# hsinnan75/GSAlign

Hardware: AMD Instinct MI355X
Metric: aligned query Gbp/s (whole node) (higher is better)
Workload: dtype u8; 1 GPU; full-human-sized pair (BASELINE configs[4]): 24 contigs with GRCh38 chromosome lengths, 3.08 Gbp, repeat injection, vs 1; inflight_contexts_per_gpu=8, world_size=1, parallelism=one GPU

## Files before the change

### gsalign_amd/capi.py

```python
from __future__ import annotations

import ctypes as C
import os
import subprocess

import numpy as np

HERE = os.path.dirname(os.path.abspath(__file__))
LIB_PATH = os.path.join(HERE, "lib", "libgsa_hip.so")

EXPORTS = [
    "gsa_default_params", "gsa_create", "gsa_create_opts", "gsa_reserve_index", "gsa_release_reserved", "gsa_clone", "gsa_clone_to_device", "gsa_host_alloc", "gsa_host_free", "gsa_destroy", "gsa_set_params", "gsa_last_error", "gsa_align_contig", "gsa_align_many", "gsa_align_bundle",
    "gsa_align_contig_device", "gsa_set_query_device", "gsa_device_alloc", "gsa_device_free", "gsa_device_upload", "gsa_get_seed_stats", "gsa_hit_buffers", "gsa_seed_chunks", "gsa_hit_count", "gsa_export_hits", "gsa_import_hits", "gsa_finish_contig",
    "gsa_set_query", "gsa_rewind", "gsa_run_to", "gsa_seed_count", "gsa_get_seeds", "gsa_group_count", "gsa_get_groups", "gsa_get_blocks",
    "gsa_bwt_search_batch", "gsa_ksw2_batch", "gsa_gap_similarity_batch", "gsa_get_counters", "gsa_get_timings", "gsa_set_profiling", "gsa_bind_host_thread",
    "gsa_prefetch_contig", "gsa_prefetch_bundle", "gsa_cancel_prefetch", "gsa_get_wall_sums", "gsa_get_alloc_stats", "gsa_debug_buffers", "gsa_set_option", "gsa_host_register", "gsa_host_unregister",
    "gsa_call_variants", "gsa_align_many_variants", "gsa_get_variant_timing",
    "gsa_block_cigars", "gsa_get_cigar_timing", "gsa_align_many_ex",
    "gsa_block_cs", "gsa_get_cs_timing", "gsa_extras_cs",
    "gsa_lift_set", "gsa_lift", "gsa_get_lift_timing", "gsa_extras_lift",
    "gsa_track_set", "gsa_ref_track", "gsa_get_track_timing", "gsa_extras_track",
    "gsa_block_segs", "gsa_get_seg_timing", "gsa_extras_segs",
    "gsa_proj_open", "gsa_proj_close", "gsa_proj_clear", "gsa_project", "gsa_proj_fetch", "gsa_proj_merge", "gsa_get_proj_timing",
    "gsa_index_sizes", "gsa_build_index", "gsa_get_index_build_stats",
    "gsa_create_from_pac", "gsa_export_index_table",
]


class IndexView(C.Structure):
    _fields_ = [("primary", C.c_uint64), ("L2", C.c_uint64 * 5), ("bwt", C.POINTER(C.c_uint32)), ("bwt_words", C.c_uint64),
                ("sa", C.POINTER(C.c_uint64)), ("n_sa", C.c_uint64), ("ref", C.c_char_p), ("G", C.c_int64),
                ("chr_len", C.POINTER(C.c_int32)), ("n_chr", C.c_int32)]


class Params(C.Structure):
    _fields_ = [("min_seed_len", C.c_int32), ("max_indel", C.c_int32), ("min_block_score", C.c_int32), ("min_aln_len", C.c_int32),
                ("min_identity", C.c_int32), ("sensitive", C.c_int32), ("one_on_one", C.c_int32)]


class Seed(C.Structure):
    _fields_ = [("qpos", C.c_int32), ("len", C.c_int32), ("rpos", C.c_int64)]


class Frag(C.Structure):
    _fields_ = [("bseed", C.c_int32), ("qpos", C.c_int32), ("qlen", C.c_int32), ("rlen", C.c_int32), ("rpos", C.c_int64),
                ("aln_off", C.c_int64), ("aln_len", C.c_int32), ("_pad", C.c_int32)]


class Block(C.Structure):
    _fields_ = [("score", C.c_int32), ("aln_len", C.c_int32), ("bdup", C.c_int32), ("n_frag", C.c_int32), ("frag_off", C.c_int64),
                ("bdir", C.c_int32), ("gpos", C.c_int32), ("chr", C.c_int32), ("_pad", C.c_int32)]


class Rec(C.Structure):
    _fields_ = [("w0", C.c_int32), ("w1", C.c_int32), ("w2", C.c_int32), ("w3", C.c_uint32)]


class Result(C.Structure):
    _fields_ = [("n_blocks", C.c_int32), ("n_frags", C.c_int64), ("n_aln", C.c_int64), ("blocks", C.POINTER(Block)),
                ("recs", C.POINTER(Rec)), ("aln1", C.POINTER(C.c_char)), ("aln2", C.POINTER(C.c_char))]


class Variant(C.Structure):
    _fields_ = [("rpos", C.c_int64), ("qpos", C.c_int32), ("len", C.c_int32), ("chr", C.c_int32), ("pos", C.c_int32), ("kind", C.c_int32), ("block", C.c_int32)]


class Variants(C.Structure):
    _fields_ = [("n", C.c_int64), ("v", C.POINTER(Variant)), ("n_snv", C.c_int64), ("n_ins", C.c_int64), ("n_del", C.c_int64)]


VARIANT_DT = np.dtype([("rpos", "<i8"), ("qpos", "<i4"), ("len", "<i4"), ("chr", "<i4"), ("pos", "<i4"), ("kind", "<i4"), ("block", "<i4")])
VCF_TYPE = ("SUBSTITUTE", "INSERT", "DELETE", "INSERT", "DELETE")


def variants_array(var: "Variants"):
    n = int(var.n)
    V = np.ctypeslib.as_array(C.cast(var.v, C.POINTER(C.c_uint8)), shape=(n * VARIANT_DT.itemsize,)).view(VARIANT_DT).copy() if n else np.zeros(0, VARIANT_DT)
    return V, (int(var.n_snv), int(var.n_ins), int(var.n_del))


def variant_alleles(V: np.ndarray, ref, query) -> list:
    ref = ref.tobytes() if isinstance(ref, np.ndarray) else bytes(ref)
    query = query.tobytes() if isinstance(query, np.ndarray) else bytes(query)
    out = []
    for v in V:
        r, q, n, k = int(v["rpos"]), int(v["qpos"]), int(v["len"]) + 1, int(v["kind"])
        if k == 1:
            out.append((ref[r:r + 1], query[q:q + n]))
        elif k == 2:
            out.append((ref[r:r + n], query[q:q + 1]))
        elif k == 3:
            out.append((query[q:q + 1], query[q:q + n]))
        elif k == 4:
            out.append((ref[r:r + n], ref[r:r + 1]))
        else:
            out.append((ref[r:r + 1], query[q:q + 1]))
    return out


class BlockCigar(C.Structure):
    _fields_ = [("cig_off", C.c_int64), ("n_cig", C.c_int32), ("n_eq", C.c_int32), ("n_x", C.c_int32), ("n_ins", C.c_int32), ("n_del", C.c_int32), ("_pad", C.c_int32)]


class Cigars(C.Structure):
    _fields_ = [("n_blocks", C.c_int32), ("n_ops", C.c_int64), ("blk", C.POINTER(BlockCigar)), ("ops", C.POINTER(C.c_uint32))]


class Extras(C.Structure):
    _fields_ = [("var", C.POINTER(Variants)), ("cig", C.POINTER(Cigars))]


class CsBlock(C.Structure):
    _fields_ = [("cs_off", C.c_int64), ("n_cs", C.c_int32), ("_pad", C.c_int32)]


class Cs(C.Structure):
    _fields_ = [("n_blocks", C.c_int32), ("n_bytes", C.c_int64), ("blk", C.POINTER(CsBlock)), ("cs", C.POINTER(C.c_char))]


class LiftHit(C.Structure):
    _fields_ = [("idx", C.c_int32), ("qpos", C.c_int32), ("block", C.c_int32), ("cls", C.c_uint8), ("rev", C.c_uint8), ("n_cover", C.c_uint16)]


class Lifts(C.Structure):
    _fields_ = [("n_hits", C.c_int64), ("hits", C.POINTER(LiftHit))]


class TrackWin(C.Structure):
    _fields_ = [("chr", C.c_int32), ("start", C.c_int32), ("len", C.c_int32), ("n_cov", C.c_uint32), ("n_eq", C.c_uint32), ("n_x", C.c_uint32), ("n_del", C.c_uint32), ("n_ins", C.c_uint32)]


class Tracks(C.Structure):
    _fields_ = [("n_win", C.c_int64), ("win", C.POINTER(TrackWin))]


class Seg(C.Structure):
    _fields_ = [("size", C.c_int32), ("dt", C.c_int32), ("dq", C.c_int32)]


class SegBlock(C.Structure):
    _fields_ = [("seg_off", C.c_int64), ("n_seg", C.c_int32), ("_pad", C.c_int32)]


class Segs(C.Structure):
    _fields_ = [("n_blocks", C.c_int32), ("n_segs", C.c_int64), ("blk", C.POINTER(SegBlock)), ("seg", C.POINTER(Seg))]


SEG_DT = np.dtype([("size", "<i4"), ("dt", "<i4"), ("dq", "<i4")])
SEG_BLOCK_DT = np.dtype([("seg_off", "<i8"), ("n_seg", "<i4"), ("_pad", "<i4")])
TRACK_WIN_DT = np.dtype([("chr", "<i4"), ("start", "<i4"), ("len", "<i4"), ("n_cov", "<u4"), ("n_eq", "<u4"), ("n_x", "<u4"), ("n_del", "<u4"), ("n_ins", "<u4")])
LIFT_HIT_DT = np.dtype([("idx", "<i4"), ("qpos", "<i4"), ("block", "<i4"), ("cls", "u1"), ("rev", "u1"), ("n_cover", "<u2")])
BLOCK_CS_DT = np.dtype([("cs_off", "<i8"), ("n_cs", "<i4"), ("_pad", "<i4")])
BLOCK_CIGAR_DT = np.dtype([("cig_off", "<i8"), ("n_cig", "<i4"), ("n_eq", "<i4"), ("n_x", "<i4"), ("n_ins", "<i4"), ("n_del", "<i4"), ("_pad", "<i4")])
CIGAR_LETTERS = "MIDNSHP=X"
WANT_VARIANTS, WANT_CIGARS, WANT_CS, WANT_LIFT, WANT_TRACK, WANT_SEGS, WANT_PROJ = 1, 2, 4, 16, 32, 64, 128
PROJ_NO_DUP = 1
PROJ_LETTERS = "nACGTN-"


class ProjStat(C.Structure):
    _fields_ = [("n_blocks", C.c_int32), ("_pad", C.c_int32), ("n_cols", C.c_int64)]


def lifts_array(l: "Lifts"):
    n = int(l.n_hits)
    return np.ctypeslib.as_array(C.cast(l.hits, C.POINTER(C.c_uint8)), shape=(n * LIFT_HIT_DT.itemsize,)).view(LIFT_HIT_DT).copy() if n else np.zeros(0, LIFT_HIT_DT)
# ... 107 lines not shown
        if fn.argtypes is None:
            fn.argtypes = None
    return lib


def index_sizes(G: int):
    lib = load_library()
    lib.gsa_index_sizes.argtypes = [C.c_int64, C.POINTER(C.c_uint64), C.POINTER(C.c_uint64)]
    bw, ns = C.c_uint64(), C.c_uint64()
    rc = lib.gsa_index_sizes(int(G), C.byref(bw), C.byref(ns))
    if rc != 0:
        raise GsaError(f"gsa_index_sizes -> {rc}: {lib.gsa_last_error(None).decode()}")
    return int(bw.value), int(ns.value)


BUILD_INDEX_ARGTYPES = [C.c_int, C.c_void_p, C.c_int64, C.POINTER(C.c_uint64), C.POINTER(C.c_uint64), C.c_void_p, C.c_void_p]


def build_index_arrays(pac, G: int, device: int = 0):
    lib = load_library()
    lib.gsa_build_index.argtypes = BUILD_INDEX_ARGTYPES
    pac = np.ascontiguousarray(pac, dtype=np.uint8)
    if G <= 0 or pac.size < (G + 3) // 4:
        raise ValueError("pac holds fewer than G bases")
    bw, ns = index_sizes(G)
    bwt = np.zeros(bw, np.uint32); sa = np.zeros(ns, np.uint64)
    primary = C.c_uint64(); L2 = (C.c_uint64 * 5)()
    rc = lib.gsa_build_index(int(device), C.c_void_p(pac.ctypes.data), int(G), C.byref(primary), L2, C.c_void_p(bwt.ctypes.data), C.c_void_p(sa.ctypes.data))
    if rc != 0:
        e = GsaError(f"gsa_build_index -> {rc}: {lib.gsa_last_error(None).decode()}"); e.code = rc
        raise e
    return np.array([primary.value, L2[1], L2[2], L2[3], L2[4]], dtype=np.uint64), bwt, sa


def index_build_stats():
    lib = load_library()
    ms, rounds = C.c_double(), C.c_int32()
    lib.gsa_get_index_build_stats.argtypes = [C.POINTER(C.c_double), C.POINTER(C.c_int32)]
    lib.gsa_get_index_build_stats(C.byref(ms), C.byref(rounds))
    return float(ms.value), int(rounds.value)


def bind_host_thread(device: int = 0) -> None:
    lib = load_library()
    lib.gsa_bind_host_thread.argtypes = [C.c_int]
    lib.gsa_bind_host_thread(int(device))


RESULT_FN = C.CFUNCTYPE(C.c_int, C.c_void_p, C.c_int32, C.POINTER(Result))
RESULT_VAR_FN = C.CFUNCTYPE(C.c_int, C.c_void_p, C.c_int32, C.POINTER(Result), C.POINTER(Variants))
RESULT_EX_FN = C.CFUNCTYPE(C.c_int, C.c_void_p, C.c_int32, C.POINTER(Result), C.POINTER(Extras))


class DeviceContig:

    def __init__(self, lib, device: int, seq: np.ndarray):
        seq = np.ascontiguousarray(seq, dtype=np.uint8)
        self.lib, self.device, self.size = lib, int(device), int(seq.size)
        self.ptr = lib.gsa_device_alloc(self.device, self.size)
        if not self.ptr:
            raise GsaError("gsa_device_alloc failed")
        if lib.gsa_device_upload(self.device, C.c_void_p(self.ptr), C.c_void_p(seq.ctypes.data), self.size) != 0:
            raise GsaError("gsa_device_upload failed")

    def free(self):
        if self.ptr:
            self.lib.gsa_device_free(self.device, C.c_void_p(self.ptr)); self.ptr = None


def align_many(aligners, contigs, on_result=None, in_order: bool = False, bundle: bool = True, prefetch: bool = True, variants: bool = False, cigars: bool = False, cs: bool = False, lift: bool = False, track: bool = False, segs: bool = False, proj: bool = False) -> None:
    lib = aligners[0].lib
    n = len(contigs)
    ctxs = (C.c_void_p * len(aligners))(*[a.ctx for a in aligners])
    on_dev = n > 0 and isinstance(contigs[0], DeviceContig)
    qs = (C.c_char_p * n)(*[C.cast(c.ptr if on_dev else c.ctypes.data, C.c_char_p) for c in contigs])
    ql = (C.c_int32 * n)(*[int(c.size) for c in contigs])
    flags = (1 if in_order else 0) | (2 if on_dev else 0) | (0 if bundle else 8) | (0 if prefetch else 16)
    if cigars or cs or lift or track or segs or proj:
        lib.gsa_extras_cs.argtypes = [C.POINTER(Extras), C.POINTER(Cs)]
        lib.gsa_extras_lift.argtypes = [C.POINTER(Extras), C.POINTER(Lifts)]
        lib.gsa_extras_track.argtypes = [C.POINTER(Extras), C.POINTER(Tracks)]
        lib.gsa_extras_segs.argtypes = [C.POINTER(Extras), C.POINTER(Segs)]

        def ex_cb(user, ci, res, ex):
            e = ex.contents
            args = (ci, res.contents, e.var.contents if e.var else None, e.cig.contents if e.cig else None)
            if cs:
                s = Cs()
                rc_cs = lib.gsa_extras_cs(ex, C.byref(s))
                if rc_cs != 0:
                    return int(rc_cs)
                args += (s,)
            if lift:
                lf = Lifts()
                rc_l = lib.gsa_extras_lift(ex, C.byref(lf))
                if rc_l != 0:
                    return int(rc_l)
                args += (lf,)
            if track:
                tk = Tracks()
                rc_t = lib.gsa_extras_track(ex, C.byref(tk))
                if rc_t != 0:
                    return int(rc_t)
                args += (tk,)
            if segs:
                sg = Segs()
                rc_g = lib.gsa_extras_segs(ex, C.byref(sg))
                if rc_g != 0:
                    return int(rc_g)
                args += (sg,)
            return int((on_result(*args) if on_result else 0) or 0)
        cbx = RESULT_EX_FN(ex_cb)
        lib.gsa_align_many_ex.argtypes = [C.POINTER(C.c_void_p), C.c_int32, C.POINTER(C.c_char_p), C.POINTER(C.c_int32), C.c_int32, C.c_uint32, C.c_uint32, RESULT_EX_FN, C.c_void_p]
        rc = lib.gsa_align_many_ex(ctxs, len(aligners), qs, ql, n, flags, (WANT_CIGARS if cigars or cs else 0) | (WANT_CS if cs else 0) | (WANT_VARIANTS if variants else 0) | (WANT_LIFT if lift else 0) | (WANT_TRACK if track else 0) | (WANT_SEGS if segs else 0) | (WANT_PROJ if proj else 0), cbx, None)
    elif variants:
        cbv = RESULT_VAR_FN(lambda user, ci, res, var: int((on_result(ci, res.contents, var.contents) if on_result else 0) or 0))
        lib.gsa_align_many_variants.argtypes = [C.POINTER(C.c_void_p), C.c_int32, C.POINTER(C.c_char_p), C.POINTER(C.c_int32), C.c_int32, C.c_uint32, RESULT_VAR_FN, C.c_void_p]
        rc = lib.gsa_align_many_variants(ctxs, len(aligners), qs, ql, n, flags, cbv, None)
    else:
        cb = RESULT_FN((lambda user, ci, res: int(on_result(ci, res.contents) or 0)) if on_result else 0)
        lib.gsa_align_many.argtypes = [C.POINTER(C.c_void_p), C.c_int32, C.POINTER(C.c_char_p), C.POINTER(C.c_int32), C.c_int32, C.c_uint32, RESULT_FN, C.c_void_p]
        rc = lib.gsa_align_many(ctxs, len(aligners), qs, ql, n, flags, cb, None)
    if rc != 0:
        msgs = [lib.gsa_last_error(a.ctx).decode() for a in aligners]
        raise GsaError(f"gsa_align_many{'_ex' if cigars or cs or lift or track or segs or proj else '_variants' if variants else ''} -> {rc}: {'; '.join(m for m in msgs if m)}")


def _p(a, t):
    return a.ctypes.data_as(C.POINTER(t))


def result_as_dump(r: dict, with_aln: bool = False) -> dict:
    B, F = r["blocks"], r["frags"]
    idx = np.concatenate([np.arange(o, o + n) for o, n in zip(B["frag_off"], B["n_frag"])]) if B.size else np.zeros(0, np.int64)
    Fo = F[idx] if idx.size else np.zeros(0, FRAG_DT)
    out = {"b_score": B["score"].copy(), "b_aln_len": B["aln_len"].copy(), "b_bdup": B["bdup"].copy(), "b_nfrag": B["n_frag"].copy(),
           "b_bdir": B["bdir"].copy(), "b_gpos": B["gpos"].copy(), "b_chr": B["chr"].copy(),
           "f_bseed": Fo["bseed"].copy(), "f_qpos": Fo["qpos"].copy(), "f_qlen": Fo["qlen"].copy(), "f_rlen": Fo["rlen"].copy(),
           "f_alnlen": Fo["aln_len"].copy(), "f_rpos": Fo["rpos"].copy()}
    if with_aln:
        segs1 = [r["aln1"][o:o + n] for o, n in zip(Fo["aln_off"], Fo["aln_len"]) if n]
        segs2 = [r["aln2"][o:o + n] for o, n in zip(Fo["aln_off"], Fo["aln_len"]) if n]
        out["aln1"] = np.concatenate(segs1) if segs1 else np.zeros(0, np.uint8)
        out["aln2"] = np.concatenate(segs2) if segs2 else np.zeros(0, np.uint8)
    return out


class GsaError(RuntimeError):
    pass


class Aligner:

    ENV_OPTIONS = ("split_min", "bundle_contig", "bundle_cap", "seed_budget", "dp_lane", "seed_mode", "pd_bitmap", "walk_chain_min", "pd_two_level_min", "pres_from_kmer", "pd_bytes", "sweep_shape", "dp_side", "dp_safe", "dp_fake_timeout")

    def _options_from_env(self):
        for name in self.ENV_OPTIONS:
            v = os.environ.get("GSA_" + name.upper())
            if v is not None and v != "":
                self.set_option(name, {"sweep": 0, "spec": 1, "search": 2}.get(v, v) if name == "seed_mode" else v)
        if os.environ.get("GSA_NO_PDBITMAP"):
            self.set_option("pd_bitmap", 0)

    def set_option(self, name: str, value) -> None:
        self._ck(self.lib.gsa_set_option(self.ctx, name.encode(), C.c_int64(int(value))))

    def __init__(self, idx, device: int = 0, wide: bool = False, kmer_k: int = 0, pac=None, _clone_of=None, _copy_to=None, **params):
        self.lib = load_library()
        self.idx = idx
        self._pinned = []
        self._devbufs = []
        if _clone_of is not None and _copy_to is not None:
            self.ctx = C.c_void_p()
            rc = self.lib.gsa_clone_to_device(_clone_of.ctx, int(_copy_to), C.byref(self.ctx))
            if rc != 0:
                raise GsaError(f"gsa_clone_to_device -> {rc}: {self.lib.gsa_last_error(None).decode()}")
            self._options_from_env()
            return
        if _clone_of is not None:
            self.ctx = C.c_void_p()
            rc = self.lib.gsa_clone(_clone_of.ctx, C.byref(self.ctx))
            if rc != 0:
                raise GsaError(f"gsa_clone -> {rc}: {self.lib.gsa_last_error(None).decode()}")
            self._parent = _clone_of
            self._options_from_env()
            return
        self._ref = np.ascontiguousarray(idx.ref)
        v = IndexView()
        v.primary = int(idx.hdr[0])
        v.L2[0] = 0
        for i in range(1, 5):
            v.L2[i] = int(idx.hdr[i])
        v.bwt = _p(idx.bwt, C.c_uint32); v.bwt_words = idx.bwt.size
        v.sa = _p(idx.sa, C.c_uint64); v.n_sa = idx.sa.size
        v.ref = self._ref.ctypes.data_as(C.c_char_p); v.G = idx.G
        if pac is not None:
            self._pac = np.ascontiguousarray(pac, dtype=np.uint8)
            assert self._pac.size >= (idx.G + 3) // 4
            v.ref = self._pac.ctypes.data_as(C.c_char_p)
        v.chr_len = _p(idx.chr_len, C.c_int32); v.n_chr = len(idx.chr_len)
        self.ctx = C.c_void_p()
        p = self._params(**params)
        wide = wide or os.environ.get("GSA_FORCE_WIDE", "0") not in ("", "0")
        kmer_k = kmer_k or int(os.environ.get("GSA_KMER_K", "0") or 0)
        prio = int(os.environ.get("GSA_PRIO", "0") or 0)
        flags = (1 if wide else 0) | ((kmer_k & 15) << 8) | ((prio & 3) << 16) | (4 if pac is not None else 0)
        rc = self.lib.gsa_create_opts(device, C.byref(v), C.byref(p), flags, C.byref(self.ctx))
        if rc != 0:
            e = GsaError(f"gsa_create -> {rc}: {self.lib.gsa_last_error(None).decode()}"); e.code = rc
            raise e
        self._options_from_env()

    @classmethod
    def from_reference(cls, pac, G: int, chr_len, device: int = 0, wide: bool = False, kmer_k: int = 0, **params) -> "Aligner":
        self = cls.__new__(cls)
        self.lib = load_library()
        self.idx = None
        self._pinned = []
        self._devbufs = []
        self.lib.gsa_create_from_pac.argtypes = [C.c_int, C.c_void_p, C.c_int64, C.c_void_p, C.c_int32, C.POINTER(Params), C.c_uint32, C.POINTER(C.c_void_p)]
        pac = np.ascontiguousarray(pac, dtype=np.uint8); chr_len = np.ascontiguousarray(chr_len, dtype=np.int32)
        wide = wide or os.environ.get("GSA_FORCE_WIDE", "0") not in ("", "0")
        kmer_k = kmer_k or int(os.environ.get("GSA_KMER_K", "0") or 0)
        prio = int(os.environ.get("GSA_PRIO", "0") or 0)
        flags = (1 if wide else 0) | ((kmer_k & 15) << 8) | ((prio & 3) << 16)
        self.ctx = C.c_void_p()
        p = self._params(**params)
        rc = self.lib.gsa_create_from_pac(int(device), C.c_void_p(pac.ctypes.data), int(G), C.c_void_p(chr_len.ctypes.data), int(chr_len.size), C.byref(p), flags, C.byref(self.ctx))
        if rc != 0:
            e = GsaError(f"gsa_create_from_pac -> {rc}: {self.lib.gsa_last_error(None).decode()}"); e.code = rc
            raise e
        self._options_from_env()
        return self

    TABLES = {"header": 0, "occ": 1, "occ_base": 2, "sa_dense": 3, "sa": 4, "kmer": 5, "kmer_lo": 6, "pres": 7, "ref": 8, "ref2": 9}

    def index_table(self, which) -> np.ndarray:
        w = self.TABLES[which] if isinstance(which, str) else int(which)
        self.lib.gsa_export_index_table.argtypes = [C.c_void_p, C.c_int, C.c_void_p, C.c_uint64, C.POINTER(C.c_uint64)]
        n = C.c_uint64(0)
        self._ck(self.lib.gsa_export_index_table(self.ctx, w, None, 0, C.byref(n)))
        out = np.zeros(int(n.value), np.uint8)
        if out.size:
            self._ck(self.lib.gsa_export_index_table(self.ctx, w, C.c_void_p(out.ctypes.data), out.size, C.byref(n)))
        return out

    def clone(self) -> "Aligner":
        return Aligner(self.idx, _clone_of=self)

    def clone_to_device(self, device: int) -> "Aligner":
        return Aligner(self.idx, _clone_of=self, _copy_to=device)

    def pinned_copy(self, seq: np.ndarray) -> np.ndarray:
        seq = np.ascontiguousarray(seq, dtype=np.uint8)
        p = self.lib.gsa_host_alloc(seq.size + 64)
        if not p:
            raise GsaError("gsa_host_alloc failed")
        self._pinned.append(p)
        buf = np.ctypeslib.as_array(C.cast(p, C.POINTER(C.c_uint8)), shape=(seq.size,))
        buf[:] = seq
        return buf

    def device_copy(self, seq: np.ndarray, device: int = 0) -> DeviceContig:
        d = DeviceContig(self.lib, device, seq)
        self._devbufs.append(d)
        return d

    def prefetch_contig(self, seq: np.ndarray):
        self._ck(self.lib.gsa_prefetch_contig(self.ctx, seq.ctypes.data_as(C.c_char_p), C.c_int32(seq.size)))

    def cancel_prefetch(self):
        self._ck(self.lib.gsa_cancel_prefetch(self.ctx))

    def align_contig_device(self, d: DeviceContig) -> dict:
        res = Result()
        self._ck(self.lib.gsa_align_contig_device(self.ctx, C.c_void_p(d.ptr), C.c_int32(d.size), C.byref(res)))
        return self._result(res)

    def seed_stats(self) -> np.ndarray:
        st = np.zeros(8, np.uint64)
        self._ck(self.lib.gsa_get_seed_stats(self.ctx, _p(st, C.c_uint64)))
        return st

    def _params(self, slen=15, ind=25, clr=200, alen=200, idy=70, sen=0, one=0) -> Params:
        return Params(slen, ind, clr, alen, idy, sen, one)

    def _ck(self, rc):
        if rc != 0:
            raise GsaError(f"libgsa_hip error {rc}: {self.lib.gsa_last_error(self.ctx).decode()}")

    def set_params(self, **params):
        p = self._params(**params)
        self._ck(self.lib.gsa_set_params(self.ctx, C.byref(p)))

    def set_profiling(self, on: bool, count_blocks: bool = False, seed_only: bool = False, variants: bool = False):
        self._ck(self.lib.gsa_set_profiling(self.ctx, (1 if on else 0) | (2 if count_blocks else 0) | (4 if seed_only else 0) | (8 if variants else 0)))

    def set_query(self, seq: np.ndarray):
        seq = np.ascontiguousarray(seq, dtype=np.uint8)
        self._q = seq
        self._ck(self.lib.gsa_set_query(self.ctx, seq.ctypes.data_as(C.c_char_p), C.c_int32(seq.size)))

    def rewind(self):
        self._ck(self.lib.gsa_rewind(self.ctx))

    def run_to(self, stage: int):
        self._ck(self.lib.gsa_run_to(self.ctx, stage))

    def align_contig(self, seq: np.ndarray) -> dict:
        seq = np.ascontiguousarray(seq, dtype=np.uint8)
        self._q = seq
        res = Result()
        self._ck(self.lib.gsa_align_contig(self.ctx, seq.ctypes.data_as(C.c_char_p), C.c_int32(seq.size), C.byref(res)))
        return self._result(res)

    def seed_chunks(self, seq: np.ndarray, chunk_beg: int, chunk_end: int) -> int:
        seq = np.ascontiguousarray(seq, dtype=np.uint8)
        self._q = seq
        self._ck(self.lib.gsa_seed_chunks(self.ctx, seq.ctypes.data_as(C.c_char_p), C.c_int32(seq.size), C.c_int32(chunk_beg), C.c_int32(chunk_end)))
        return int(self.lib.gsa_hit_count(self.ctx))

    def hit_count(self) -> int:
        return int(self.lib.gsa_hit_count(self.ctx))

    def export_hits(self, keys_ptr=None, vals_ptr=None):
        n = int(self.lib.gsa_hit_count(self.ctx))
        if keys_ptr is not None:
            self._ck(self.lib.gsa_export_hits(self.ctx, C.c_void_p(keys_ptr), C.c_void_p(vals_ptr)))
            return n
        k = np.zeros(n, np.uint64); v = np.zeros(n, np.uint32)
        if n:
            self._ck(self.lib.gsa_export_hits(self.ctx, C.c_void_p(k.ctypes.data), C.c_void_p(v.ctypes.data)))
        return k, v

    def import_hits(self, keys, vals, n=None):
        if n is None:
            keys = np.ascontiguousarray(keys, np.uint64); vals = np.ascontiguousarray(vals, np.uint32)
            n = int(keys.size); kp, vp = keys.ctypes.data, vals.ctypes.data
        else:
            kp, vp = keys, vals
        self._ck(self.lib.gsa_import_hits(self.ctx, C.c_void_p(kp), C.c_void_p(vp), C.c_int64(n)))

    def finish_contig(self) -> dict:
        res = Result()
        self._ck(self.lib.gsa_finish_contig(self.ctx, C.byref(res)))
        return self._result(res)

    def seeds(self):
        n = self.lib.gsa_seed_count(self.ctx)
        out = np.zeros(n, dtype=SEED_DT)
        if n:
            self._ck(self.lib.gsa_get_seeds(self.ctx, out.ctypes.data_as(C.c_void_p)))
        return out["qpos"].copy(), out["len"].copy(), out["rpos"].copy()

    def groups(self):
        n = self.lib.gsa_group_count(self.ctx)
        b = np.zeros(n, np.int32); e = np.zeros(n, np.int32)
        if n:
            self._ck(self.lib.gsa_get_groups(self.ctx, _p(b, C.c_int32), _p(e, C.c_int32)))
        return b, e

    def _result(self, res: Result) -> dict:
        nb, nf, na = res.n_blocks, res.n_frags, res.n_aln
        blocks = np.ctypeslib.as_array(C.cast(res.blocks, C.POINTER(C.c_uint8)), shape=(nb * BLOCK_DT.itemsize,)).view(BLOCK_DT).copy() if nb else np.zeros(0, BLOCK_DT)
        recs = np.ctypeslib.as_array(C.cast(res.recs, C.POINTER(C.c_uint8)), shape=(nf * REC_DT.itemsize,)).view(REC_DT).copy() if nf else np.zeros(0, REC_DT)
        frags = expand_recs(recs)
        a1 = np.ctypeslib.as_array(C.cast(res.aln1, C.POINTER(C.c_uint8)), shape=(na,)).copy() if na else np.zeros(0, np.uint8)
        a2 = np.ctypeslib.as_array(C.cast(res.aln2, C.POINTER(C.c_uint8)), shape=(na,)).copy() if na else np.zeros(0, np.uint8)
        return dict(blocks=blocks, frags=frags, aln1=a1, aln2=a2)

    def call_variants(self, k: int = 0):
        var = Variants()
        self.lib.gsa_call_variants.argtypes = [C.c_void_p, C.c_int32, C.POINTER(Variants)]
        self._ck(self.lib.gsa_call_variants(self.ctx, C.c_int32(k), C.byref(var)))
        return variants_array(var)

    def block_cigars(self, k: int = 0):
        cig = Cigars()
        self.lib.gsa_block_cigars.argtypes = [C.c_void_p, C.c_int32, C.POINTER(Cigars)]
        self._ck(self.lib.gsa_block_cigars(self.ctx, C.c_int32(k), C.byref(cig)))
        return cigars_arrays(cig)

    def block_cs(self, k: int = 0):
        cs = Cs()
        self.lib.gsa_block_cs.argtypes = [C.c_void_p, C.c_int32, C.POINTER(Cs)]
        self._ck(self.lib.gsa_block_cs(self.ctx, C.c_int32(k), C.byref(cs)))
        return cs_arrays(cs)

    def lift_set(self, pos) -> None:
        pos = np.ascontiguousarray(pos, dtype=np.int64)
        self.lib.gsa_lift_set.argtypes = [C.c_void_p, C.c_void_p, C.c_int64]
        self._ck(self.lib.gsa_lift_set(self.ctx, C.c_void_p(pos.ctypes.data) if pos.size else None, C.c_int64(pos.size)))

    def lift(self, k: int = 0):
        l = Lifts()
        self.lib.gsa_lift.argtypes = [C.c_void_p, C.c_int32, C.POINTER(Lifts)]
        self._ck(self.lib.gsa_lift(self.ctx, C.c_int32(k), C.byref(l)))
        return lifts_array(l)

    def lift_timing(self):
        ms, n = C.c_double(0), C.c_int64(0)
        self.lib.gsa_get_lift_timing.argtypes = [C.c_void_p, C.POINTER(C.c_double), C.POINTER(C.c_int64)]
        self._ck(self.lib.gsa_get_lift_timing(self.ctx, C.byref(ms), C.byref(n)))
        return float(ms.value), int(n.value)

    def track_set(self, window: int) -> None:
        self.lib.gsa_track_set.argtypes = [C.c_void_p, C.c_int32]
        self._ck(self.lib.gsa_track_set(self.ctx, C.c_int32(int(window))))

    def track(self, k: int = 0):
        t = Tracks()
        self.lib.gsa_ref_track.argtypes = [C.c_void_p, C.c_int32, C.POINTER(Tracks)]
        self._ck(self.lib.gsa_ref_track(self.ctx, C.c_int32(k), C.byref(t)))
        return tracks_array(t)

    def track_timing(self):
        ms, n = C.c_double(0), C.c_int64(0)
        self.lib.gsa_get_track_timing.argtypes = [C.c_void_p, C.POINTER(C.c_double), C.POINTER(C.c_int64)]
        self._ck(self.lib.gsa_get_track_timing(self.ctx, C.byref(ms), C.byref(n)))
        return float(ms.value), int(n.value)

    def block_segs(self, k: int = 0):
        sg = Segs()
        self.lib.gsa_block_segs.argtypes = [C.c_void_p, C.c_int32, C.POINTER(Segs)]
        self._ck(self.lib.gsa_block_segs(self.ctx, C.c_int32(k), C.byref(sg)))
        return segs_arrays(sg)

    def seg_timing(self):
        ms, n = C.c_double(0), C.c_int64(0)
        self.lib.gsa_get_seg_timing.argtypes = [C.c_void_p, C.POINTER(C.c_double), C.POINTER(C.c_int64)]
        self._ck(self.lib.gsa_get_seg_timing(self.ctx, C.byref(ms), C.byref(n)))
        return float(ms.value), int(n.value)

    def proj_open(self, share: "Aligner" = None, no_dup: bool = False) -> None:
        self.lib.gsa_proj_open.argtypes = [C.c_void_p, C.c_void_p, C.c_uint32]
        self._ck(self.lib.gsa_proj_open(self.ctx, share.ctx if share is not None else None, C.c_uint32(PROJ_NO_DUP if no_dup else 0)))
# ... 160 lines not shown
```

### gsalign_amd/csrc/gsa_api.hip

```cpp
#include <cstring>
#include "gsa_ctx.h"

void collect_events(gsa_ctx *c)
{
	if (!c->profiling && !c->prof_seed) { c->ev_pending = 0; return; }
	float ms;
	if ((c->ev_pending & 1) && !c->profiling) {
		if (hipEventElapsedTime(&ms, c->ev[0], c->ev[1]) == hipSuccess) {
			c->kernel_ms[0] = ms;
			c->acc_seed_ms += ms;
		}
	} else {
		if (c->ev_pending & 1) {
			if (hipEventElapsedTime(&ms, c->ev[0], c->ev[1]) == hipSuccess) c->kernel_ms[0] = ms;
			if (hipEventElapsedTime(&ms, c->ev[1], c->ev[2]) == hipSuccess) c->kernel_ms[1] = ms;
			if (hipEventElapsedTime(&ms, c->ev[2], c->ev[3]) == hipSuccess) c->kernel_ms[2] = ms;
		}
		if (c->ev_pending & 2) { if (hipEventElapsedTime(&ms, c->ev[4], c->ev[5]) == hipSuccess) c->kernel_ms[3] = ms; }
	}
	c->ev_pending = 0;
	(void)hipGetLastError();
}

static int rewind_to_hits(gsa_ctx *c)
// ... 260 lines not shown
	if (n >= (1ll << 31) - 256) return gsa_fail(c, GSA_ERR_LIMIT, "gsa_lift_set: too many positions");
	for (int64_t i = 0; i < n; i++) if (pos[i] < 0 || pos[i] >= c->G)
		return gsa_fail(c, GSA_ERR_ARG, "gsa_lift_set: position " + std::to_string((long long)pos[i]) + " (entry " + std::to_string((long long)i) + ") lies outside the reference [0, " + std::to_string((long long)c->G) + ")");
	if (n == 0) { c->lift_n = 0; return GSA_OK; }
	GSA_CHECK(c, hipSetDevice(c->device));
	c->lift_n = 0;
	ENS(i64, d_lpos, (size_t)n);
	const hipError_t e = hipMemcpy(c->d_lpos.p, pos, (size_t)n * sizeof(i64), hipMemcpyHostToDevice);
	if (e != hipSuccess) { return gsa_fail(c, GSA_ERR_HIP, std::string("gsa_lift_set (hipMemcpy H2D): ") + hipGetErrorString(e)); }
	c->lift_n = n;
	return GSA_OK;
}
int gsa_lift(gsa_ctx *c, int32_t k, gsa_lifts *out) { return lift_call(c, k, out); }
int gsa_get_lift_timing(gsa_ctx *c, double *ms_sum, int64_t *n_calls) { return pass_timing(c, &gsa_ctx::lift_ms_sum, &gsa_ctx::lift_calls, ms_sum, n_calls); }

int gsa_track_set(gsa_ctx *c, int32_t window)
{
	if (!c) return GSA_ERR_ARG;
	if (window < 0) return gsa_fail(c, GSA_ERR_ARG, "gsa_track_set: the window is negative");
	i64 nwin = 0;
	if (window > 0) for (size_t i = 0; i < c->h_chr_len.size(); i++) nwin += ((i64)c->h_chr_len[i] + window - 1) / window;
	if (nwin >= (1ll << 31) - 256) return gsa_fail(c, GSA_ERR_LIMIT, "gsa_track_set: " + std::to_string((long long)nwin) + " windows (2^31 - 256 or more)");
	c->track_w = window; c->track_nwin = nwin;
	return GSA_OK;
}
int gsa_ref_track(gsa_ctx *c, int32_t k, gsa_tracks *out) { return track_call(c, k, out); }
int gsa_get_track_timing(gsa_ctx *c, double *ms_sum, int64_t *n_calls) { return pass_timing(c, &gsa_ctx::track_ms_sum, &gsa_ctx::track_calls, ms_sum, n_calls); }

int gsa_block_segs(gsa_ctx *c, int32_t k, gsa_segs *out) { return segs_call(c, k, out, nullptr, nullptr); }
int gsa_get_seg_timing(gsa_ctx *c, double *ms_sum, int64_t *n_calls) { return pass_timing(c, &gsa_ctx::seg_ms_sum, &gsa_ctx::seg_calls, ms_sum, n_calls); }

int gsa_proj_open(gsa_ctx *c, gsa_ctx *share, uint32_t flags) { return c ? proj_open(c, share, flags) : GSA_ERR_ARG; }
int gsa_proj_close(gsa_ctx *c)
{
	if (!c) return GSA_ERR_ARG;
	if (!c->proj) return gsa_fail(c, GSA_ERR_STATE, "gsa_proj_close: no accumulator (gsa_proj_open first)");
	return proj_release(c);
}
int gsa_proj_clear(gsa_ctx *c)
{
	if (!c) return GSA_ERR_ARG;
	if (!c->proj) return gsa_fail(c, GSA_ERR_STATE, "gsa_proj_clear: no accumulator (gsa_proj_open first)");
	return proj_clear(c);
}
int gsa_project(gsa_ctx *c, int32_t k, gsa_proj_stat *out) { return proj_call(c, k, out); }
static int proj_range_ready(gsa_ctx *c, int64_t p0, int64_t n, const char *who)
{
	if (!c) return GSA_ERR_ARG;
	if (!c->proj) return gsa_fail(c, GSA_ERR_STATE, std::string(who) + ": no accumulator (gsa_proj_open first)");
	if (n < 0 || p0 < 0 || p0 > c->proj->G || n > c->proj->G - p0) return gsa_fail(c, GSA_ERR_ARG, std::string(who) + ": the range lies outside the reference [0, " + std::to_string((long long)c->proj->G) + ")");
	return GSA_OK;
}
int gsa_proj_fetch(gsa_ctx *c, int64_t p0, int64_t n, char *text, uint32_t *words)
{
	if (const int rc = proj_range_ready(c, p0, n, "gsa_proj_fetch")) return rc;
	return (n == 0 || (!text && !words)) ? GSA_OK : proj_fetch(c, p0, n, text, words);
}
int gsa_proj_merge(gsa_ctx *c, int64_t p0, int64_t n, const uint32_t *words)
{
	if (const int rc = proj_range_ready(c, p0, n, "gsa_proj_merge")) return rc;
	if (n == 0) return GSA_OK;
	return words ? proj_merge(c, p0, n, words) : GSA_ERR_ARG;
}
int gsa_get_proj_timing(gsa_ctx *c, double *ms_sum, int64_t *n_calls) { return pass_timing(c, &gsa_ctx::proj_ms_sum, &gsa_ctx::proj_calls, ms_sum, n_calls); }

int gsa_get_wall_sums(gsa_ctx *c, double ms[10], int64_t *n)
{
	if (!c || !ms || !n) return GSA_ERR_ARG;
	memcpy(ms, c->wall_ms, sizeof(c->wall_ms)); *n = c->wall_n;
	if (c->up && c->own_up) { std::lock_guard<std::mutex> g(c->up->mu); ms[9] = c->up->jobs ? c->up->copy_ms / (double)c->up->jobs * (double)c->wall_n : 0.0; }
	return GSA_OK;
}
int gsa_get_alloc_stats(gsa_ctx *c, double *ms, int64_t *n, int64_t *bytes)
{
	if (!c) return GSA_ERR_ARG;
	if (ms) *ms = c->alloc_ms; if (n) *n = c->alloc_n; if (bytes) *bytes = c->alloc_bytes;
	return GSA_OK;
}

int gsa_set_profiling(gsa_ctx *c, int enable)
{
	if (!c) return GSA_ERR_ARG;
	c->acc_seed_ms = 0.0;
	memset(c->wall_ms, 0, sizeof(c->wall_ms));
	c->wall_n = 0;
	if (c->up && c->own_up) {
		std::lock_guard<std::mutex> g(c->up->mu);
		c->up->copy_ms = c->up->wait_ms = c->up->bytes = 0;
		c->up->jobs = 0;
	}
	c->var_ms_sum = 0;
	c->var_calls = 0;
	c->prof_var = (enable & 8) != 0;
	c->profiling = (enable & 1) != 0;
	c->count_blocks = (enable & 2) != 0;
	c->prof_seed = (enable & 4) != 0;
	return GSA_OK;
}

int64_t gsa_seed_count(gsa_ctx *c) { return c ? c->n_seeds : 0; }
int gsa_get_seeds(gsa_ctx *c, gsa_seed *out)
{
	if (!c || (!out && c->n_seeds)) return GSA_ERR_ARG;
	if (c->stage < 1) return gsa_fail(c, GSA_ERR_STATE, "run stage 1 first");
	const size_t n = (size_t)c->n_seeds; if (!n) return GSA_OK;
	{ int rc = seed_view_sort(c); if (rc) return rc; GSA_CHECK(c, hipStreamSynchronize(c->stream)); }
	std::vector<i32> q(n), l(n); std::vector<i64> r(n);
	GSA_CHECK(c, hipMemcpy(q.data(), c->s_q.p, n * 4, hipMemcpyDeviceToHost));
	GSA_CHECK(c, hipMemcpy(l.data(), c->s_len.p, n * 4, hipMemcpyDeviceToHost));
	GSA_CHECK(c, hipMemcpy(r.data(), c->s_r.p, n * 8, hipMemcpyDeviceToHost));
	for (size_t i = 0; i < n; i++) { out[i].qpos = q[i]; out[i].len = l[i]; out[i].rpos = r[i]; }
	return GSA_OK;
}
int gsa_group_count(gsa_ctx *c)
{
	if (!c) return 0;
	if (c->n_groups < 0) {
		if (seed_view_sort(c) != GSA_OK) return 0;
		hipStreamSynchronize(c->stream);
		i32 ng = 0;
		if (hipMemcpy(&ng, c->d_mail.as<i32>() + M_NG, 4, hipMemcpyDeviceToHost) != hipSuccess) return 0;
		c->n_groups = ng;
	}
	return c->n_groups;
}
int gsa_get_groups(gsa_ctx *c, int32_t *beg, int32_t *end)
{
	if (!c) return GSA_ERR_ARG;
	if (c->stage < 1) return gsa_fail(c, GSA_ERR_STATE, "run stage 1 first");
	const size_t ng = (size_t)gsa_group_count(c); if (!ng) return GSA_OK;
	std::vector<i32> gb(ng + 1);
	GSA_CHECK(c, hipMemcpy(gb.data(), c->g_beg.p, (ng + 1) * 4, hipMemcpyDeviceToHost));
	for (size_t i = 0; i < ng; i++) { beg[i] = gb[i]; end[i] = gb[i + 1]; }
	return GSA_OK;
}
int gsa_get_blocks(gsa_ctx *c, gsa_result *out)
{
	if (!c || !out) return GSA_ERR_ARG;
	if (c->stage < 2) return gsa_fail(c, GSA_ERR_STATE, "run stage 2 first");
	if (c->bnd.n && c->stage < 8) return gsa_fail(c, GSA_ERR_STATE, "gsa_get_blocks: the context holds a bundle -- only its finished result (gsa_align_bundle's out[]) is defined per contig");
	if (c->frags_stage != c->stage) { int rc = build_block_view(c); if (rc) return rc; }
	out->n_blocks = (int32_t)c->h_blocks.size(); out->blocks = c->h_blocks.data();
	if (c->result_pinned && c->stage == 8) {
		out->n_frags = c->n_frags; out->n_aln = c->n_aln;
		out->recs = c->p_frags.as<gsa_rec>(); out->aln1 = c->h_taln1; out->aln2 = c->h_taln2;
	} else {
		out->n_frags = (int64_t)c->h_frags.size(); out->n_aln = (int64_t)c->h_aln1.size();
		out->recs = c->h_frags.data(); out->aln1 = c->h_aln1.data(); out->aln2 = c->h_aln2.data();
	}
	return GSA_OK;
}
int gsa_get_counters(gsa_ctx *c, uint64_t counters[8]) { if (!c) return GSA_ERR_ARG; memcpy(counters, c->counters, sizeof(c->counters)); return GSA_OK; }
int gsa_get_timings(gsa_ctx *c, float ms[8]) { if (!c) return GSA_ERR_ARG; memcpy(ms, c->kernel_ms, sizeof(c->kernel_ms)); if (c->prof_seed && !c->profiling) ms[6] = (float)c->acc_seed_ms; return GSA_OK; }
int gsa_get_seed_stats(gsa_ctx *c, uint64_t st[8]) { if (!c) return GSA_ERR_ARG; memcpy(st, c->dbg, sizeof(c->dbg)); return GSA_OK; }
}
```

### gsalign_amd/csrc/gsa_create.hip

```cpp
#include <algorithm>
#include <cstring>
#include <pthread.h>
#include <sched.h>
#include "gsa_ctx.h"

static thread_local std::string g_create_error;
int gsa_fail(gsa_ctx *ctx, int code, const std::string &msg)
{
	if (ctx) ctx->err = msg; else g_create_error = msg;
	return code;
}

static int ctx_abandon(gsa_ctx *c, int rc, const std::string &msg = std::string())
{
	if (!msg.empty()) g_create_error = msg; else if (!c->err.empty()) g_create_error = c->err;
	gsa_destroy(c);
	return rc;
}

static int create_device_ok(const char *who, int device)
{
	int ndev = 0;
	if (hipGetDeviceCount(&ndev) != hipSuccess || ndev <= 0) { (void)hipGetLastError(); return gsa_fail(nullptr, GSA_ERR_HIP, "no HIP device available (libgsa_hip.so has no CPU path)"); }
	if (device < 0 || device >= ndev) return gsa_fail(nullptr, GSA_ERR_ARG, std::string(who) + ": bad device ordinal");
// ... 284 lines not shown
	(void)hipSetDeviceFlags(hipDeviceScheduleSpin); (void)hipGetLastError();
	gsa_ctx *c = new gsa_ctx();
	c->device = device; c->force_wide = parent->force_wide; c->prio_mode = parent->prio_mode; c->seed_budget = parent->seed_budget; c->opt = parent->opt;
	if (int rc = ctx_private_init(c)) return ctx_abandon(c, rc);
	struct Pair { const DevBuf *src; DevBuf *dst; };
	std::vector<Pair> tab = { { &own->d_bwt, &c->d_bwt }, { &own->d_occ_base, &c->d_occ_base }, { &own->d_sa, &c->d_sa }, { &own->d_ref, &c->d_ref }, { &own->d_chr_end, &c->d_chr_end },
		{ &own->d_chr_of_end, &c->d_chr_of_end }, { &own->d_sa_dense, &c->d_sa_dense }, { &own->d_kmer, &c->d_kmer }, { &own->d_ref2, &c->d_ref2 } };
	for (gsa_ctx *src = parent; src; src = src->lender) {
		if (!c->d_pres.cap && src->d_pres.p && (const void *)parent->di.pres == src->d_pres.p) { tab.push_back({ &src->d_pres, &c->d_pres }); c->d_pres.cap = 1; }
		if (!c->d_kmer_lo.cap && src->d_kmer_lo.p && (const void *)parent->di.kmer_lo == src->d_kmer_lo.p) { tab.push_back({ &src->d_kmer_lo, &c->d_kmer_lo }); c->d_kmer_lo.cap = 1; }
	}
	c->d_pres.cap = c->d_kmer_lo.cap = 0;
	for (const Pair &t : tab) {
		if (!t.src->p) continue;
		const size_t bytes = t.src->len ? t.src->len : t.src->cap;
		if (bytes == 0) return ctx_abandon(c, GSA_ERR_STATE, "gsa_clone_to_device: an index table of unknown size");
		if (hipMalloc(&t.dst->p, bytes + 256) != hipSuccess) { (void)hipGetLastError(); return ctx_abandon(c, GSA_ERR_NOMEM, "gsa_clone_to_device: hipMalloc of an index table"); }
		t.dst->cap = bytes + 256; t.dst->len = bytes;
		const hipError_t e = (device == own->device) ? hipMemcpyAsync(t.dst->p, t.src->p, bytes, hipMemcpyDeviceToDevice, c->stream)
		                                             : hipMemcpyPeerAsync(t.dst->p, device, t.src->p, own->device, bytes, c->stream);
		if (e != hipSuccess) return ctx_abandon(c, GSA_ERR_HIP, std::string("gsa_clone_to_device: device-to-device copy: ") + hipGetErrorString(e));
	}
	c->di = parent->di;
	auto move_ptr = [&](const void *p) -> const void * {
		if (!p) return nullptr;
		for (const Pair &t : tab) if (t.src->p && (const char *)p >= (const char *)t.src->p && (const char *)p < (const char *)t.src->p + (t.src->len ? t.src->len : t.src->cap)) return (const char *)t.dst->p + ((const char *)p - (const char *)t.src->p);
		return (const void *)~(uintptr_t)0;
	};
	bool lost = false;
#define MOVE(field, T) do { const void *q_ = move_ptr((const void *)c->di.field); if (q_ == (const void *)~(uintptr_t)0) lost = true; c->di.field = (T)q_; } while (0)
	MOVE(bwt, const uint4 *); MOVE(occ_base, const u64 *); MOVE(sa, const u64 *); MOVE(sa32, const u32 *); MOVE(sa64, const u64 *); MOVE(ref, const uint8_t *); MOVE(ref2, const u32 *);
	MOVE(chr_end, const i64 *); MOVE(chr_of_end, const i32 *); MOVE(kmer, const u64 *); MOVE(kmer_lo, const u64 *); MOVE(pres, const u32 *);
#undef MOVE
	if (lost) return ctx_abandon(c, GSA_ERR_STATE, "gsa_clone_to_device: an index pointer outside the tables of its owner");
	c->G = parent->G;
	c->h_chr_end = parent->h_chr_end; c->h_chr_fwd = parent->h_chr_fwd; c->h_chr_of_end = parent->h_chr_of_end; c->h_chr_len = parent->h_chr_len;
	c->prm = parent->prm;
	if (hipStreamSynchronize(c->stream) != hipSuccess) return ctx_abandon(c, GSA_ERR_HIP, "gsa_clone_to_device: waiting for the copies");
	*out = c;
	return GSA_OK;
}

int gsa_reserve_index(int device, uint64_t seq_len, uint32_t flags)
{
	int ndev = 0;
	if (hipGetDeviceCount(&ndev) != hipSuccess || device < 0 || device >= ndev || seq_len == 0) { (void)hipGetLastError(); return GSA_ERR_ARG; }
	if (hipSetDevice(device) != hipSuccess) return GSA_ERR_HIP;
	const bool wide = (flags & GSA_CREATE_WIDE) != 0 || seq_len >= 0xFFFFFFF0ull;
	size_t want[2];
	want[0] = ((size_t)seq_len + 1 + 32) * (wide ? 8 : 4) + 256;
	{
		int k = 0; while ((1ull << (2 * k)) < seq_len) k++;
		k += 2; if (k > 15) k = 15;
		size_t fr = 0, tot = 0; if (hipMemGetInfo(&fr, &tot) != hipSuccess) { (void)hipGetLastError(); fr = 8ull << 30; }
		const size_t esz = wide ? 32 : 16;
		while (k > 2 && ((size_t)esz << (2 * k)) > fr / 4) k--;
		const int kk = (int)((flags >> 8) & 15u); if (kk >= 2 && kk <= 15 && ((size_t)esz << (2 * kk)) <= fr / 2) k = kk;
		want[1] = k >= 2 ? ((size_t)esz << (2 * k)) : 0;
	}
	gsa_release_reserved(device);
	for (int k = 0; k < 2; k++) {
		if (!want[k]) continue;
		void *p = nullptr;
		if (hipMalloc(&p, want[k]) != hipSuccess) { (void)hipGetLastError(); continue; }
		std::lock_guard<std::mutex> g(g_res_mu);
		g_res[device & 63][k].p = p; g_res[device & 63][k].bytes = want[k];
	}
	return GSA_OK;
}
void gsa_release_reserved(int device)
{
	void *f[2] = { nullptr, nullptr };
	{ std::lock_guard<std::mutex> g(g_res_mu); for (int k = 0; k < 2; k++) { f[k] = g_res[device & 63][k].p; g_res[device & 63][k].p = nullptr; g_res[device & 63][k].bytes = 0; } }
	if (f[0] || f[1]) { (void)hipSetDevice(device); for (int k = 0; k < 2; k++) if (f[k]) hipFree(f[k]); }
}

static bool device_local_cpus(int device, cpu_set_t *set)
{
	char bus[64] = { 0 };
	if (hipDeviceGetPCIBusId(bus, (int)sizeof(bus) - 1, device) != hipSuccess) { (void)hipGetLastError(); return false; }
	for (char *p = bus; *p; p++) if (*p >= 'A' && *p <= 'Z') *p = (char)(*p - 'A' + 'a');
	char path[160]; snprintf(path, sizeof(path), "/sys/bus/pci/devices/%s/local_cpulist", bus);
	FILE *f = fopen(path, "r"); if (!f) return false;
	char line[4096]; const bool got = fgets(line, sizeof(line), f) != nullptr; fclose(f);
	if (!got) return false;
	CPU_ZERO(set); int n = 0;
	for (char *p = line; *p;) {
		while (*p == ',' || *p == ' ' || *p == '\n') p++;
		if (!*p) break;
		char *e; long a = strtol(p, &e, 10), b = a; if (e == p) break;
		if (*e == '-') { p = e + 1; b = strtol(p, &e, 10); if (e == p) break; }
		for (long k = a; k <= b && k < CPU_SETSIZE; k++) { CPU_SET((int)k, set); n++; }
		p = e;
	}
	return n > 0;
}
int gsa_bind_host_thread(int device)
{
	cpu_set_t set;
	if (!device_local_cpus(device, &set)) return GSA_OK;
	(void)pthread_setaffinity_np(pthread_self(), sizeof(set), &set);
	return GSA_OK;
}

void *gsa_host_alloc(size_t bytes)
{
	void *p = nullptr;
	if (hipHostMalloc(&p, bytes ? bytes : 1) != hipSuccess) { (void)hipGetLastError(); return nullptr; }
	return p;
}
void gsa_host_free(void *p) { if (p) (void)hipHostFree(p); }
int gsa_host_register(void *p, size_t bytes)
{
	if (!p || !bytes) return GSA_ERR_ARG;
	if (hipHostRegister(p, bytes, hipHostRegisterDefault) != hipSuccess) { (void)hipGetLastError(); return GSA_ERR_HIP; }
	return GSA_OK;
}
int gsa_host_unregister(void *p)
{
	if (!p) return GSA_ERR_ARG;
	if (hipHostUnregister(p) != hipSuccess) { (void)hipGetLastError(); return GSA_ERR_HIP; }
	return GSA_OK;
}

void *gsa_device_alloc(int device, size_t bytes)
{
	void *p = nullptr;
	if (hipSetDevice(device) != hipSuccess || hipMalloc(&p, (bytes ? bytes : 1) + 64) != hipSuccess) { (void)hipGetLastError(); return nullptr; }
	return p;
}
void gsa_device_free(int device, void *p) { if (p && hipSetDevice(device) == hipSuccess) (void)hipFree(p); }
int gsa_device_upload(int device, void *dst, const void *src, size_t bytes)
{
	if (!dst || (!src && bytes)) return GSA_ERR_ARG;
	if (hipSetDevice(device) != hipSuccess || hipMemcpy(dst, src, bytes, hipMemcpyHostToDevice) != hipSuccess) { (void)hipGetLastError(); return GSA_ERR_HIP; }
	return GSA_OK;
}

int gsa_set_option(gsa_ctx *c, const char *name, int64_t value)
{
	if (!c || !name) return GSA_ERR_ARG;
	const std::string k(name);
	auto in = [&](int64_t lo, int64_t hi) { return value >= lo && value <= hi; };
	const int64_t BIG = (int64_t)1 << 40;
	if (k == "split_min") { if (!in(0, BIG)) return gsa_fail(c, GSA_ERR_ARG, "split_min: 0 .. 2^40 bases"); c->opt.split_min = value; }
	else if (k == "bundle_contig") { if (!in(0, BIG)) return gsa_fail(c, GSA_ERR_ARG, "bundle_contig: 0 (no bundles) .. 2^40 bases"); c->opt.bundle_contig = value; }
	else if (k == "bundle_cap") { if (!in(1, BIG)) return gsa_fail(c, GSA_ERR_ARG, "bundle_cap: 1 .. 2^40 bases"); c->opt.bundle_cap = value; }
	else if (k == "seed_budget") { if (!in(1, 0xffffffffll)) return gsa_fail(c, GSA_ERR_ARG, "seed_budget: 1 .. 2^32 - 1 wave-iterations"); c->seed_budget = (u32)value; }
	else if (k == "dp_lane") { if (!in(0, 1 << 20)) return gsa_fail(c, GSA_ERR_ARG, "dp_lane: 0 (no lane class: one per wavefront) .. 2^20 cells"); c->opt.dp_lane = (int)value; }
	else if (k == "seed_mode") { if (value < 0 || value > 2) return gsa_fail(c, GSA_ERR_ARG, "seed_mode: 0 sweep, 1 speculative, 2 search"); c->opt.seed_mode = (int)value; }
	else if (k == "seed_lhop") { if (value != 0 && (!in(16, 1 << 16) || (value & (value - 1)))) return gsa_fail(c, GSA_ERR_ARG, "seed_lhop: 0 or a power of two >= 16"); c->opt.seed_lhop = (int)value; }
	else if (k == "pd_bitmap") c->opt.pd_bitmap = value != 0;
	else if (k == "dp_side") c->opt.dp_side = value != 0;
	else if (k == "pd_two_level_min") { if (!in(0, BIG)) return gsa_fail(c, GSA_ERR_ARG, "pd_two_level_min: >= 0 blocks"); c->opt.pd_two_level_min = value; }
	else if (k == "pd_bytes") { if (!in(0, 2)) return gsa_fail(c, GSA_ERR_ARG, "pd_bytes: 0 never, 1 by the hit count, 2 always"); c->opt.pd_bytes = (int)value; }
	else if (k == "pres_from_kmer") c->opt.pres_from_kmer = value != 0;
	else if (k == "walk_chain_min") { if (!in(0, BIG)) return gsa_fail(c, GSA_ERR_ARG, "walk_chain_min: >= 0 seeds"); c->opt.walk_chain_min = value; }
	else if (k == "sweep_shape") { if (value < -1 || value > 1) return gsa_fail(c, GSA_ERR_ARG, "sweep_shape: -1, 0 or 1"); c->opt.sweep_shape = (int)value; }
	else if (k == "dp_safe") c->dp_safe = value != 0;
	else if (k == "dp_fake_timeout") { if (!in(0, 1 << 20)) return gsa_fail(c, GSA_ERR_ARG, "dp_fake_timeout: >= 0"); c->dp_fake_timeout = (int)value; }
	else return gsa_fail(c, GSA_ERR_ARG, "gsa_set_option: unknown option " + k);
	return GSA_OK;
}

int gsa_debug_buffers(gsa_ctx *c, int top)
{
	if (!c) return GSA_ERR_ARG;
	struct E { const char *name; size_t cap, len; };
	std::vector<E> v;
#define X(n) if (c->n.p) v.push_back({ #n, c->n.cap, c->n.len });
	GSA_DEVBUFS(X)
#undef X
	std::sort(v.begin(), v.end(), [](const E &a, const E &b) { return a.cap > b.cap; });
	size_t tot = 0; for (const E &e : v) tot += e.cap;
	fprintf(stderr, "[gsa_debug_buffers] %zu device buffers, %.2f GB held\n", v.size(), (double)tot / 1e9);
	for (size_t k = 0; k < v.size() && (int)k < top; k++) fprintf(stderr, "  %-16s %10.1f MB held  %10.1f MB asked\n", v[k].name, (double)v[k].cap / 1e6, (double)v[k].len / 1e6);
	return GSA_OK;
}

int gsa_index_sizes(int64_t G, uint64_t *bwt_words, uint64_t *n_sa)
{
	if (G <= 0 || !bwt_words || !n_sa) return gsa_fail(nullptr, GSA_ERR_ARG, "gsa_index_sizes: bad argument");
	const uint64_t S = 2 * (uint64_t)G;
	*bwt_words = (S + 15) / 16 + ((S + 127) / 128 + 1) * 8;
	*n_sa = (S + 32) / 32;
	return GSA_OK;
}
static thread_local double g_ix_ms = 0; static thread_local int32_t g_ix_rounds = 0;
int gsa_build_index(int device, const uint8_t *pac, int64_t G, uint64_t *primary, uint64_t L2[5], uint32_t *bwt, uint64_t *sa)
{
	if (!pac || !primary || !L2 || !bwt || !sa || G <= 0) return gsa_fail(nullptr, GSA_ERR_ARG, "gsa_build_index: bad argument");
	if (2 * G + 1 > (1ll << 31) - 2) return gsa_fail(nullptr, GSA_ERR_LIMIT, "gsa_build_index: the reference is longer than 1 073 741 822 bases (the device builder sorts 32-bit suffix indices)");
	if (int rc = create_device_ok("gsa_build_index", device)) return rc;
	gsa_ctx *c = new gsa_ctx();
	c->device = device;
	hipError_t e = hipSetDevice(device);
	if (e == hipSuccess) e = hipStreamCreate(&c->stream);
	if (e == hipSuccess) e = hipMalloc(&c->d_mail.p, MAIL_N * sizeof(i32));
	if (e == hipSuccess) { c->d_mail.cap = MAIL_N * sizeof(i32); e = hipMemset(c->d_mail.p, 0, MAIL_N * sizeof(i32)); }
	if (e != hipSuccess) { (void)hipGetLastError(); return ctx_abandon(c, GSA_ERR_HIP, std::string("gsa_build_index: device set-up: ") + hipGetErrorString(e)); }
	double ms = 0; int32_t rounds = 0;
	if (int rc = build_index_device(c, pac, G, primary, L2, bwt, sa, &ms, &rounds)) { g_create_error = c->err; return ctx_abandon(c, rc); }
	g_ix_ms = ms; g_ix_rounds = rounds;
	gsa_destroy(c);
	return GSA_OK;
}
int gsa_get_index_build_stats(double *ms, int32_t *rounds)
{
	if (!ms || !rounds) return GSA_ERR_ARG;
	*ms = g_ix_ms; *rounds = g_ix_rounds;
	return GSA_OK;
}
}
```

### gsalign_amd/csrc/gsa_ctx.h

```cpp
#ifndef GSA_CTX_H
#define GSA_CTX_H
#include <atomic>
#include <chrono>
#include <condition_variable>
#include <deque>
#include <mutex>
#include <thread>
#include "gsa_internal.h"

struct Leaf {
	i32 beg, end;
	i32 sumlen;
	i32 q_first, q_last_end;
	i64 r_first, r_last_end;
	i32 blk;
	i32 cut4, cut5;
	i32 blk_score;
};

enum { M_NB = 0, M_NC = 1, M_NBLK = 2, M_NG = 3, M_NR = 4, M_NJ = 5, M_NL = 6, M_LBERR = 7, M_ANY = 8, M_NLANE = 40, M_TICKET = 48, M_NBRAW = 49, M_NR2 = 50, M_NF = 51, M_NJOB = 52, M_OPSTOT = 53, M_NALN = 54, M_DPERR = 64, M_NLARGE = 65, M_DPERR2 = 66, M_CELLS = 68  , M_DPERR3 = 41, M_LBDONE = 42, M_LFSTEPS = 44 , M_NEARLY = 62, M_EOPS = 63, M_NTOUCH = 46 , M_MAXBLK = 56 , MAIL_N = 72 };
#define LEAF_CHUNK 1024

struct HostBlock {
	i32 leaf_beg, leaf_end;
	i32 score;
	i32 bdup;
	i32 aln_len, bdir, gpos, chr;
};

struct QuerySlot {
	DevBuf d_query;
	DevBuf d_bndtab, p_bndtab;
	std::vector<i32> b_off, b_qlen;
	std::vector<const char *> src;
	i32 n = 0;
	i32 lmax = 0; i64 tot = 0; size_t o_cc = 0, o_src = 0;
	bool pending = false;
	std::atomic<int> busy{0};
	std::atomic<int> up_err{0};
};
static inline void slot_wait(QuerySlot &s) { while (s.busy.load(std::memory_order_acquire) > 0) std::this_thread::yield(); }

struct Uploader {
	struct Piece { void *dst; const void *src; size_t n; };
	struct Job { std::vector<Piece> pieces; std::atomic<int> *busy; std::atomic<int> *err; std::chrono::steady_clock::time_point t_push; };
	double copy_ms = 0, wait_ms = 0, bytes = 0; long long jobs = 0;
	int device = 0; hipStream_t st = nullptr;
	std::thread th; std::mutex mu; std::condition_variable cv; std::deque<Job> q; bool stop = false;
	size_t n_demand = 0;
	void run();
	void push(Job &&j) { j.busy->fetch_add(1); j.t_push = std::chrono::steady_clock::now(); { std::lock_guard<std::mutex> g(mu); q.push_back(std::move(j)); } cv.notify_one(); }
};

struct Options {
	int64_t split_min = 20000000;
	int64_t bundle_contig = 16000000;
	int64_t bundle_cap = 64000000;
	int dp_lane = 512;
	int seed_lhop = 0;
	int seed_mode = 1;
	int pd_bitmap = 1;
	int sweep_shape = -1;
	int dp_side = 0;
	int64_t walk_chain_min = 100000;
	int64_t pd_two_level_min = 2000000;
	int pd_bytes = 1;
	int pres_from_kmer = 1;
	int kmer_k = 0;
};

struct ProjAcc { u32 *words = nullptr; i64 G = 0; int device = 0; std::atomic<int> refs{1}; std::atomic<int> dirty{0}; };

struct gsa_ctx {
	int device = 0;
	Options opt;
	Uploader *up = nullptr; bool own_up = false;
	hipStream_t stream = nullptr;
	hipStream_t stream_seed = nullptr;
	hipEvent_t ev_seed_fork = nullptr;
	u64 seed_ticket = 0;
	int n_cus = 0;
	bool seed_lds_checked = false;
	hipStream_t stream_aux[4] = {nullptr, nullptr, nullptr, nullptr};
	std::string err;
	Params prm;
	DevIndex di = {};
	gsa_ctx *index_owner = nullptr;
	gsa_ctx *lender = nullptr;
	std::atomic<int> n_borrowers{0};
	int prio_mode = 0;
	bool force_wide = false;
	bool profiling = false;
	bool prof_seed = false;
	bool count_blocks = false;
	u64 dbg[8] = {0, 0, 0, 0, 0, 0, 0, 0};
	hipEvent_t ev[28] = {};
	float kernel_ms[8] = {};
	double wall_ms[10] = {0, 0, 0, 0, 0, 0, 0, 0, 0, 0}; int64_t wall_n = 0;
	double acc_seed_ms = 0.0;
	u64 counters[8] = {};

	DevBuf d_bwt, d_bwt_ref, d_occ_base, d_sa, d_ref, d_chr_end, d_chr_of_end;
	std::vector<i64> h_chr_end, h_chr_fwd; std::vector<i32> h_chr_of_end, h_chr_len;
	i64 G = 0;

	QuerySlot qs[2]; int q_cur = -1;
	i32 qlen = 0; int stage = 0;
	const uint8_t *q_dev = nullptr;
	bool split = false; i64 rng_beg = 0, rng_end = 0;
	int qbits = 1, pdbits = 1;
	i64 pd_span = 0;

	Bundle bnd = { 0, 0, 0, nullptr, nullptr }; bool bundle_call = false;
	std::vector<i32> b_off, b_qlen;
	std::vector<std::vector<HostBlock> > b_lists;
	std::vector<i32> b_blk0;
	DevBuf d_bblk, p_bblk, p_ba0;
	std::vector<i32> b_nblk; std::vector<i64> b_frag0;

	DevBuf tmp;
	DevBuf leaf[9];
	DevBuf d_cnt; u64 *h_cnt = nullptr;
	DevBuf d_mail; i32 *h_mail = nullptr;
	DevBuf d_lb_status[2]; u32 lb_epoch = 0, lb_base = 0;
	DevBuf p_leaf;
	int ev_pending = 0;
	bool s2_host = false;

	DevBuf d_ref2;
	DevBuf d_kmer;
	DevBuf d_kmer_lo;
	DevBuf d_pres;
	DevBuf d_sa_dense;
	DevBuf d_cand_s, d_cand_len, d_cand_x0, d_cand_freq, d_onpath, d_cand_cnt;
	size_t cand_cap_per_chunk = 1536;
	DevBuf d_heavy, dn_lf, dn_x0;
	bool seed_sweep_next = false, seed_sweep_probe = false; int seed_sweep_run = 0, seed_sweep_period = 8;
	u32 seed_budget = 256;
	DevBuf d_chunk_hits, d_chunk_base;
	DevBuf d_key_a, d_key_b, d_val_a, d_val_b;
	i64 n_seeds = 0; bool hits_sorted = false;
	DevBuf s_q, s_len, s_r, s_gid;
	DevBuf d_flag, d_scan;
	i32 n_groups = 0;
	bool pd_path = false, seed_view_ready = false, pdbm_dirty = true; i64 pd_words = 0;
	DevBuf w_j0; u32 walk_ticket = 0, walk_epoch = 0;
	DevBuf d_zero;
	DevBuf d_pdby; bool pd_bytes = false;
	DevBuf d_pdcb;
	DevBuf d_pdbm, d_gpre, d_key_c, d_val_c;
	DevBuf g_beg;

	i64 n_a = 0;
	DevBuf a_q, a_len, a_r, a_gb, a_ge;
	DevBuf a_uniq, a_cu, a_alive, a_ws, a_wid;
	DevBuf a_next, a_brk, a_aurank, a_aulist, a_runinfo;
	DevBuf w_best, w_sum, w_n;
	DevBuf d_btab;
	DevBuf d_flag2, d_scan2, d_i64a;
	i64 n_b = 0, n_c = 0;
	DevBuf b_q, b_len, b_r, b_gb, b_ge;
	DevBuf c_q, c_len, c_r, c_gb, c_ge;
	DevBuf c_bid;
	i32 n_blocks2 = 0;
	DevBuf blk_beg, blk_end, blk_score;
	std::vector<i32> h_blk_beg, h_blk_end, h_blk_score;

	i64 n_r = 0;
	DevBuf r_q, r_len, r_r, r_bid, r_tmp_q, r_tmp_len, r_tmp_r, r_tmp_bid;
	DevBuf r_cut4, r_cut5, r_simjob, r_simres;
	DevBuf d_leaf; std::vector<Leaf> h_leaf;
	std::vector<HostBlock> blocks;
	std::vector<i32> h_r_q, h_r_len; std::vector<i64> h_r_r;
	bool have_host_seeds = false;

	i64 n_frags = 0, n_aln = 0;
	i32 n_large = 0;
	DevBuf p_jpatch; i32 n_jobs = 0;
	DevBuf d_tail, p_tail;
	const i32 *h_tmail = nullptr, *h_tpatch = nullptr; char *h_taln1 = nullptr, *h_taln2 = nullptr;
	i64 nf_ub = 0, span_ub = 0;
	DevBuf fb_seedbase, fb_sbeg, fb_fragbase;
	DevBuf f_rec;
	DevBuf f_rec16;
	DevBuf f_type, f_mism, f_alnlen, f_job, f_score;
	DevBuf j_frag, j_opsoff, j_nops, d_ops, j_cells;
	DevBuf d_dp_lane_order;
	DevBuf d_dp_arena;
	DevBuf d_dp_bnd, d_dp_ctr, d_dp_jobs, d_dp_large;
	DevBuf e_id, e_rec, e_list, e_off1, e_off2, e_opsoff, e_nops, e_ops, e_rev, r_head, f_early, r_orig, r_tmp_orig, p_early;
	bool early_consumed = false;
	bool early_listed = false;
	i32 n_early = 0; bool early_in_flight = false; std::vector<i32> h_early;
	bool dp_dirty = true;
	bool dp_timeout = false, dp_safe = false;
	int dp_fake_timeout = 0;
	u32 dp_epoch = 0;
	DevBuf p_dp, p_sj, p_sj_early;
	DevBuf d_alnoff;
	DevBuf bl_alnlen, bl_score;
	std::vector<gsa_rec> h_frags; std::vector<gsa_block> h_blocks; std::vector<char> h_aln1, h_aln2;
	int frags_stage = 0;
	DevBuf p_frags, p_blk; bool result_pinned = false;
	DevBuf d_vblk, d_vcnt, d_vwg, d_var, p_vblk, p_vhdr, p_var;
	bool prof_var = false; hipEvent_t ev_var[2] = {nullptr, nullptr}; double var_ms_sum = 0; long long var_calls = 0;
	DevBuf d_cblk, d_cout, d_ccnt, d_cwg, d_cpre, d_crun, d_cops, p_cblk, p_chdr, p_cout, p_cops;
	double cig_ms_sum = 0; long long cig_calls = 0;
	DevBuf d_crpos, d_cqpos, d_slen, d_swg, d_spre, d_sout, d_cs, p_shdr, p_sout, p_cs;
	double cs_ms_sum = 0; long long cs_calls = 0;
	DevBuf d_lpos, d_lblk, d_lpick, d_lwg, d_lhit, p_lblk, p_lhdr, p_lhit;
	i64 lift_n = 0;
	double lift_ms_sum = 0; long long lift_calls = 0;
	DevBuf d_tblk, d_tiv, d_tbin, d_twg, d_tout, p_tblk, p_tiv, p_thdr, p_tout;
	i32 track_w = 0; i64 track_nwin = 0;
	size_t track_zeroed = 0; bool track_dirty = false;
	double track_ms_sum = 0; long long track_calls = 0;
	DevBuf d_sgwg, d_sgpre, d_sgbnd, d_sgout, d_sgseg, p_sghdr, p_sgout, p_sgseg;
	double seg_ms_sum = 0; long long seg_calls = 0;
	ProjAcc *proj = nullptr; u32 proj_flags = 0;
	DevBuf d_pblk, d_ppre, d_pwg, d_pstage, p_pblk, p_phdr, p_pstage;
	double proj_ms_sum = 0; long long proj_calls = 0;
	double alloc_ms = 0; long long alloc_n = 0, alloc_bytes = 0;
};

#define GSA_DEVBUFS(X) \
	X(d_bwt) X(d_bwt_ref) X(d_occ_base) X(d_sa) X(d_ref) X(d_chr_end) X(d_chr_of_end) X(qs[0].d_query) X(qs[1].d_query) X(qs[0].d_bndtab) X(qs[1].d_bndtab) \
	X(tmp) X(d_cnt) X(d_zero) X(d_mail) X(d_lb_status[0]) X(d_lb_status[1]) X(d_sa_dense) X(d_kmer) X(d_kmer_lo) X(d_pres) X(d_ref2) \
	X(d_cand_s) X(d_cand_len) X(d_cand_x0) X(d_cand_freq) X(d_onpath) X(d_cand_cnt) X(d_heavy) X(dn_lf) X(dn_x0) X(d_chunk_hits) X(d_chunk_base) \
	X(d_key_a) X(d_key_b) X(d_val_a) X(d_val_b) X(s_q) X(s_len) X(s_r) X(s_gid) X(d_flag) X(d_scan) X(g_beg) X(w_j0) X(d_pdbm) X(d_pdby) X(d_pdcb) X(d_gpre) X(d_key_c) X(d_val_c) \
	X(a_q) X(a_len) X(a_r) X(a_gb) X(a_ge) X(a_uniq) X(a_cu) X(a_alive) X(a_ws) X(a_wid) X(a_next) X(a_brk) X(a_aurank) X(a_aulist) X(a_runinfo) X(w_best) X(w_sum) X(w_n) \
	X(d_btab) X(d_flag2) X(d_scan2) X(d_i64a) X(b_q) X(b_len) X(b_r) X(b_gb) X(b_ge) X(c_q) X(c_len) X(c_r) X(c_gb) X(c_ge) X(c_bid) X(blk_beg) X(blk_end) X(blk_score) \
	X(r_q) X(r_len) X(r_r) X(r_bid) X(r_tmp_q) X(r_tmp_len) X(r_tmp_r) X(r_tmp_bid) X(r_cut4) X(r_cut5) X(r_simjob) X(r_simres) X(d_leaf) \
	X(fb_seedbase) X(fb_sbeg) X(fb_fragbase) X(f_rec) X(f_rec16) X(f_type) X(f_mism) X(f_alnlen) X(f_job) X(f_score) \
	X(d_dp_lane_order) X(d_dp_bnd) X(d_dp_ctr) X(d_dp_jobs) X(d_dp_large) X(d_tail) \
	X(e_id) X(e_rec) X(e_list) X(e_off1) X(e_off2) X(e_opsoff) X(e_nops) X(e_ops) X(e_rev) X(r_head) X(f_early) X(r_orig) X(r_tmp_orig) \
	X(j_frag) X(j_opsoff) X(j_nops) X(d_ops) X(j_cells) X(d_alnoff) X(bl_alnlen) X(bl_score) X(d_bblk) X(d_dp_arena) \
	X(d_vblk) X(d_vcnt) X(d_vwg) X(d_var) X(d_cblk) X(d_cout) X(d_ccnt) X(d_cwg) X(d_cpre) X(d_crun) X(d_cops) X(d_crpos) X(d_cqpos) X(d_slen) X(d_swg) X(d_spre) X(d_sout) X(d_cs) \
	X(d_lpos) X(d_lblk) X(d_lpick) X(d_lwg) X(d_lhit) X(d_tblk) X(d_tiv) X(d_tbin) X(d_twg) X(d_tout) X(d_sgwg) X(d_sgpre) X(d_sgbnd) X(d_sgout) X(d_sgseg) X(d_pblk) X(d_ppre) X(d_pwg) X(d_pstage) \
	X(leaf[0]) X(leaf[1]) X(leaf[2]) X(leaf[3]) X(leaf[4]) X(leaf[5]) X(leaf[6]) X(leaf[7]) X(leaf[8])
#define GSA_PINBUFS(X) \
	X(p_frags) X(p_tail) X(p_leaf) X(p_blk) X(p_dp) X(p_sj) X(p_sj_early) X(p_jpatch) X(p_early) X(qs[0].p_bndtab) X(qs[1].p_bndtab) X(p_bblk) X(p_ba0) \
	X(p_vblk) X(p_vhdr) X(p_var) X(p_cblk) X(p_chdr) X(p_cout) X(p_cops) X(p_shdr) X(p_sout) X(p_cs) X(p_lblk) X(p_lhdr) X(p_lhit) X(p_tblk) X(p_tiv) X(p_thdr) X(p_tout) X(p_sghdr) X(p_sgout) X(p_sgseg) X(p_pblk) X(p_phdr) X(p_pstage)

static inline void ctx_quiesce(gsa_ctx *c)
{
	hipStreamSynchronize(c->stream);
	for (int i = 0; i < 4; i++) if (c->stream_aux[i]) hipStreamSynchronize(c->stream_aux[i]);
}

void *dev_take_reserved(int device, size_t bytes, size_t *got);
template <class T> static inline T *dev_ensure(gsa_ctx *c, DevBuf &b, size_t n, bool exact = false)
{
	size_t bytes = (n ? n : 1) * sizeof(T);
// ... 90 lines not shown
```

### gsalign_amd/csrc/k_dp_stripe.hip

```cpp
#include <algorithm>
#include "gsa_ctx.h"
#include "gsa_dp.h"

struct StripeJob { i32 job, m, n, P; i64 diroff, bndoff; i32 ctr, first_block; };
#define DP_TILE_ROWS 160
#define DP_STRIPE_BYTES(M) ((((size_t)(M) + 63 + 7) >> 3) << 8)
#define DP_C1_PAD 320
#define DP_TILE_SLACK 16
#ifndef DP_G
#define DP_G 8
#endif
#ifdef GSA_DP_TIMING
#define DPT(...) __VA_ARGS__
#else
#define DPT(...)
#endif
#define DP_LOOK 21
#define DP_WAIT_TICKS 200000000ull
#define DP_CLASS_M 768
#define DP_CLASS_TOP 1536
#define DP_CLASS_MIN_JOBS 4096
#ifndef DP_PRIO_BLOCKS
#define DP_PRIO_BLOCKS 96
#endif
#define DP_LDS_M 3968

typedef unsigned short v2u16 __attribute__((ext_vector_type(2)));
#define V2(X) __builtin_bit_cast(v2u16, (u32)(X))
#define U1(X) __builtin_bit_cast(u32, (v2u16)(X))
__device__ __forceinline__ u32 pk_add(u32 a, u32 b) { return U1(V2(a) + V2(b)); }
__device__ __forceinline__ u32 pk_sub(u32 a, u32 b) { return U1(V2(a) - V2(b)); }
__device__ __forceinline__ u32 pk_max(u32 a, u32 b) { return U1(__builtin_elementwise_max(V2(a), V2(b))); }
__device__ __forceinline__ u32 pk_min(u32 a, u32 b) { return U1(__builtin_elementwise_min(V2(a), V2(b))); }
__device__ __forceinline__ u32 pk_sub_sat(u32 a, u32 b) { return U1(__builtin_elementwise_sub_sat(V2(a), V2(b))); }
__device__ __forceinline__ u32 pk_mad(u32 a, u32 b, u32 c) { return U1(V2(a) * V2(b) + V2(c)); }
__device__ __forceinline__ u32 pk_shl(u32 a, u32 sh) { return U1(V2(a) << V2(sh)); }
#define DP_OPAQUE(X) asm volatile("" : "+v"(X))

template <int WPB>
__global__ void __launch_bounds__(64 * WPB) k_dp_stripe(const i32 *__restrict__ blk2job, const StripeJob *__restrict__ sjobs, const uint8_t *__restrict__ pool1, const i64 *__restrict__ off1,
                                                   const uint8_t *__restrict__ pool2, const i64 *__restrict__ off2, uint8_t *dirbase, u32 *bndbase, u32 *ctr,
                                                   uint8_t *revbase, uint8_t *ops, const i64 *__restrict__ ops_off, i32 *ops_len, u32 ep, i32 lds_c1, i32 lds_rows, u32 *err, i32 tick_slot)
{
	extern __shared__ __attribute__((aligned(16))) u32 C2[];
	uint8_t *tile = (uint8_t *)C2;
	__shared__ u32 s_bid, s_tick;
	if (threadIdx.x == 0) {
		s_tick = 0;
		const u32 tk = __hip_atomic_fetch_add(&ctr[tick_slot], 1u, __ATOMIC_RELAXED, __HIP_MEMORY_SCOPE_AGENT);
		if (tk == gridDim.x - 1) __hip_atomic_store(&ctr[tick_slot], 0u, __ATOMIC_RELAXED, __HIP_MEMORY_SCOPE_AGENT);
		s_bid = tk;
	}
	__syncthreads();
	const u32 bid = s_bid;
	if (bid < DP_PRIO_BLOCKS) __builtin_amdgcn_s_setprio(3);
	const StripeJob sj = sjobs[blk2job[bid]];
	const int lane = threadIdx.x & 63, wave = threadIdx.x >> 6;
	const int m = sj.m, n = sj.n, P = sj.P, PP = (P + 1) >> 1;
	const int pp = ((int)bid - sj.first_block) * WPB + wave;
	const uint8_t *s1 = pool1 + off1[sj.job], *s2 = pool2 + off2[sj.job];
	const size_t pitch = (size_t)DP_STRIPE_BYTES(m);
	const int nblk = (m + 63 + 7) >> 3;
	uint8_t *dir = dirbase + sj.diroff;
	u32 *bnd_in = bndbase + sj.bndoff + (size_t)(pp - 1) * m, *bnd_out = bndbase + sj.bndoff + (size_t)pp * m;
	{
		int fe = (m + DP_C1_PAD + 63) & ~63; fe = fe < (lds_c1 >> 2) ? fe : (lds_c1 >> 2);
		for (int t = threadIdx.x; t < fe; t += 64 * WPB) {
			const int j = t - 128, jb = j - 64;
			const u32 ca = (j >= 0 && j < m) ? (u32)gsa_nt4(s1[j]) : 4u, cb = (jb >= 0 && jb < m) ? (u32)gsa_nt4(s1[jb]) : 4u;
			C2[t] = (ca < 4 ? ca : 0x0cu) | 0x0c000c00u | ((cb < 4 ? 4u + cb : 0x0cu) << 16);
		}
	}
	u32 *lds_bnd = C2 + (lds_c1 >> 2);
	if (WPB > 1) for (int t = threadIdx.x; t < (WPB - 1) * lds_rows; t += 64 * WPB) lds_bnd[t] = 0;
	u32 *lin = lds_bnd + (size_t)(wave > 0 ? wave - 1 : 0) * lds_rows, *lout = lds_bnd + (size_t)(wave < WPB - 1 ? wave : 0) * lds_rows;
	const bool out_lds = WPB > 1 && wave < WPB - 1;
	const int tA = pp * 128 + lane, tB = tA + 64;
	const bool hasB = 2 * pp + 1 < P;
	const int WpB = !hasB ? 0 : (n - pp * 128 - 64 < 64 ? n - pp * 128 - 64 : 64);
	const int WpA = n - pp * 128 < 64 ? n - pp * 128 : 64;
	const int cqA = tA < n ? gsa_nt4(s2[tA]) : 4, cqB = tB < n ? gsa_nt4(s2[tB]) : 4;
	u32 tblA = 0, tblB = 0;
#pragma unroll
	for (int cc = 0; cc < 4; cc++) {
		tblA |= (u32)(cqA == 4 ? 0 : (cqA == cc ? 7 ^ 6 : 5 ^ 6)) << (8 * cc);
		tblB |= (u32)(cqB == 4 ? 0 : (cqB == cc ? 7 ^ 6 : 5 ^ 6)) << (8 * cc);
	}
	const u32 uinit2 = (tA ? 2u : 0u) | (2u << 16);
	u32 u2 = uinit2, y2 = 0;
	u32 bin = 0, gnext = 0;
	__syncthreads();
	if (pp >= PP) return;
	const int S_end = hasB ? 64 + m + WpB - 1 : m + WpA - 1;
	DPT(const unsigned long long T0c = wall_clock64();)
	u32 *dirA = (u32 *)(dir + (size_t)(2 * pp) * pitch), *dirB = (u32 *)(dir + (size_t)(2 * pp + 1) * pitch);
	if (pp > 0) {
		const int row = (lane & (DP_G - 1)) < m ? (lane & (DP_G - 1)) : m - 1;
		gnext = (WPB > 1 && wave > 0) ? __hip_atomic_load(&lin[row], __ATOMIC_RELAXED, __HIP_MEMORY_SCOPE_WORKGROUP) : __hip_atomic_load(&bnd_in[row], __ATOMIC_RELAXED, __HIP_MEMORY_SCOPE_AGENT);
	}
	asm volatile("" :: "v"(gnext));
	const bool pub_stripe = pp < PP - 1;
	u32 pk2 = 0;
	u32 hb = 0;
	const u32 selx = lane ? 0x0c060c04u : 0x0c040c00u, selv = lane ? 0x0c070c05u : 0x0c050c01u;
	u32 acc = 0, r0 = 0;
	u32 c1 = 0x00010001u, c2 = 0x00020002u, c4 = 0x00040004u, c7 = 0x00070007u, c16 = 0x00100010u;
	DP_OPAQUE(c1); DP_OPAQUE(c2); DP_OPAQUE(c4); DP_OPAQUE(c7); DP_OPAQUE(c16);
#define DP_WL_LIT(HB, VAL, K) asm("v_writelane_b32 %0, %1, %2" : "+v"(HB) : "s"(VAL), "n"(K));
#define DP_WL_VAR(HB, VAL, K) if (lane == (K)) HB = (VAL);
#define DP_LOADG(MODE, ROW) ((MODE) == 2 ? __hip_atomic_load(&lin[ROW], __ATOMIC_RELAXED, __HIP_MEMORY_SCOPE_WORKGROUP) : __hip_atomic_load(&bnd_in[ROW], __ATOMIC_RELAXED, __HIP_MEMORY_SCOPE_AGENT))
#define DP_STEP(K2, MODE, WSEL, GUARD, WL)                                                                       \
	{                                                                                                           \
		const int s_ = s0 + (K2);                                                                               \
		if (((K2) & (DP_G - 1)) == 0) {                                                                         \
			if ((MODE) == 0) bin = (s_ == 0 && lane == 0) ? 0u : 0x200u;     \
			else if (s_ < m) {                                                                                  \
				 \
				const int row = s_ + (lane & (DP_G - 1));                                                       \
				const bool need = lane < DP_G && row < m;                                                       \
				u32 g = gnext;                                                                                  \
				if (!__all(!need || (g >> 16) == ep)) {       \
					u32 spins = 0; const unsigned long long t_wait0 = wall_clock64();                          \
					do {                                                                                        \
						if ((++spins & 255) == 0 && (wall_clock64() - t_wait0 > DP_WAIT_TICKS || __hip_atomic_load(err, __ATOMIC_RELAXED, __HIP_MEMORY_SCOPE_AGENT))) { if (lane == 0) __hip_atomic_store(err, 1u, __ATOMIC_RELAXED, __HIP_MEMORY_SCOPE_AGENT); break; } \
						__builtin_amdgcn_s_sleep(1);                                                            \
						if (need) g = DP_LOADG(MODE, row);                                                      \
					} while (!__all(!need || (g >> 16) == ep));                                                  \
				}                                                                                               \
				bin = g & 0xffffu;                                                                              \
				 \
				const int rown = row + DP_G < m ? row + DP_G : m - 1;                                           \
				gnext = DP_LOADG(MODE, rown);                                                                   \
			}                                                                                                   \
		}                                                                                                       \
		               \
		                          \
		const u32 bin0 = (u32)__builtin_amdgcn_readlane((int)bin, (K2) & (DP_G - 1));                           \
		const u32 rot = (u32)__builtin_amdgcn_mov_dpp((int)pk2, 0x13C, 0xf, 0xf, true);                         \
		WL(hb, (u32)__builtin_amdgcn_readlane((int)pk2, 63) >> 16, (K2) & 7)       \
		const u32 x1 = __builtin_amdgcn_perm(rot, bin0, selx), v1 = __builtin_amdgcn_perm(rot, bin0, selv);     \
		const u32 z0 = __builtin_amdgcn_perm(tblB, tblA, (WSEL)) ^ 0x00060006u;                                 \
		const u32 a = pk_add(x1, v1), b = pk_add(y2, u2);                                                       \
		const u32 z1 = pk_max(z0, a), z2 = pk_max(z1, b);                                                       \
		const u32 ta = pk_min(pk_sub(z1, z0), c1), tb = pk_min(pk_sub(z2, z1), c1);       \
		const u32 zc = pk_min(z2, c7);                                                                          \
		const u32 un = pk_sub(zc, v1), vn = pk_sub(zc, u2), zz = pk_sub(zc, c2);                                \
		const u32 xa = pk_sub_sat(a, zz), yb = pk_sub_sat(b, zz);                                                \
		const u32 fa = pk_min(xa, c1), fb = pk_min(yb, c1);                                                      \
		 \
		acc = pk_mad(acc, c16, pk_mad(pk_mad(fb, c2, fa), c4, pk_mad(tb, c2, ta)));                             \
		u2 = un; y2 = yb;                                                                                       \
		pk2 = __builtin_amdgcn_perm(vn, xa, 0x06020400u);       \
		if (GUARD) {                                                                                            \
			const u32 keep = (lane <= s_ ? 0xffffu : 0u) | (lane <= s_ - 64 ? 0xffff0000u : 0u);               \
			u2 = (u2 & keep) | (uinit2 & ~keep); y2 &= keep;                                                    \
		}                                                                                                       \
		if (((K2) & 7) == 3) r0 = acc;                                                                  \
		if (((K2) & 7) == 7) {                                                                                  \
			const int blk = s_ >> 3;                                                                            \
			if (!(GUARD) || blk < nblk) dirA[((size_t)blk << 6) + lane] = __builtin_amdgcn_perm(acc, r0, 0x05040100u); \
			if (hasB && (!(GUARD) || (blk >= 8 && blk - 8 < nblk))) dirB[((size_t)(blk - 8) << 6) + lane] = __builtin_amdgcn_perm(acc, r0, 0x07060302u); \
		}                                                                                                       \
		if (((K2) & 7) == 7 && pub_stripe && s_ >= 135) {                                                       \
			   \
			const int row = s_ - 135 + lane;                                                                    \
			if (lane < 8 && row < m) {                                                                          \
				if (out_lds) __hip_atomic_store(&lout[row], (ep << 16) | hb, __ATOMIC_RELAXED, __HIP_MEMORY_SCOPE_WORKGROUP); \
				else __hip_atomic_store(&bnd_out[row], (ep << 16) | hb, __ATOMIC_RELAXED, __HIP_MEMORY_SCOPE_AGENT); \
			}                                                                                                   \
		}                                                                                                       \
	}
#define DP_LOOP(MODE)                                                                                           \
	for (int s0 = 0; s0 < S_end; s0 += 16) {                                                                    \
		const u32 *crow = C2 + 128 + s0 - lane;                                  \
		if (s0 + 16 <= S_end) {                                                                                 \
			u32 w[16];                                                                                          \
			_Pragma("unroll") for (int k2 = 0; k2 < 16; k2++) w[k2] = crow[k2];                                   \
			if (s0 >= 128 && s0 + 16 <= 8 * nblk) {                                                             \
				 \
				DP_STEP(0, MODE, w[0], 0, DP_WL_LIT) DP_STEP(1, MODE, w[1], 0, DP_WL_LIT) DP_STEP(2, MODE, w[2], 0, DP_WL_LIT) DP_STEP(3, MODE, w[3], 0, DP_WL_LIT) DP_STEP(4, MODE, w[4], 0, DP_WL_LIT) DP_STEP(5, MODE, w[5], 0, DP_WL_LIT) DP_STEP(6, MODE, w[6], 0, DP_WL_LIT) DP_STEP(7, MODE, w[7], 0, DP_WL_LIT) \
				DP_STEP(8, MODE, w[8], 0, DP_WL_LIT) DP_STEP(9, MODE, w[9], 0, DP_WL_LIT) DP_STEP(10, MODE, w[10], 0, DP_WL_LIT) DP_STEP(11, MODE, w[11], 0, DP_WL_LIT) DP_STEP(12, MODE, w[12], 0, DP_WL_LIT) DP_STEP(13, MODE, w[13], 0, DP_WL_LIT) DP_STEP(14, MODE, w[14], 0, DP_WL_LIT) DP_STEP(15, MODE, w[15], 0, DP_WL_LIT) \
			} else {                                                                                            \
				DP_STEP(0, MODE, w[0], 1, DP_WL_LIT) DP_STEP(1, MODE, w[1], 1, DP_WL_LIT) DP_STEP(2, MODE, w[2], 1, DP_WL_LIT) DP_STEP(3, MODE, w[3], 1, DP_WL_LIT) DP_STEP(4, MODE, w[4], 1, DP_WL_LIT) DP_STEP(5, MODE, w[5], 1, DP_WL_LIT) DP_STEP(6, MODE, w[6], 1, DP_WL_LIT) DP_STEP(7, MODE, w[7], 1, DP_WL_LIT) \
				DP_STEP(8, MODE, w[8], 1, DP_WL_LIT) DP_STEP(9, MODE, w[9], 1, DP_WL_LIT) DP_STEP(10, MODE, w[10], 1, DP_WL_LIT) DP_STEP(11, MODE, w[11], 1, DP_WL_LIT) DP_STEP(12, MODE, w[12], 1, DP_WL_LIT) DP_STEP(13, MODE, w[13], 1, DP_WL_LIT) DP_STEP(14, MODE, w[14], 1, DP_WL_LIT) DP_STEP(15, MODE, w[15], 1, DP_WL_LIT) \
			}                                                                                                   \
		} else {                                                                                                \
			for (int k2 = 0; s0 + k2 < S_end; k2++) DP_STEP(k2, MODE, crow[k2], 1, DP_WL_VAR)                                 \
		}                                                                                                       \
	}
	if (pp == 0) { DP_LOOP(0) } else if (WPB > 1 && wave > 0) { DP_LOOP(2) } else { DP_LOOP(1) }
#undef DP_LOOP
#undef DP_STEP
#undef DP_LOADG
	if (S_end & 7) {
		if (S_end & 3) acc = pk_shl(acc, (u32)(4 * (4 - (S_end & 3))) * 0x00010001u);
		if ((S_end & 7) < 4) r0 = acc;
		const int blk = S_end >> 3;
		if (blk < nblk) dirA[((size_t)blk << 6) + lane] = __builtin_amdgcn_perm(acc, r0, 0x05040100u);
		if (hasB && blk >= 8 && blk - 8 < nblk) dirB[((size_t)(blk - 8) << 6) + lane] = __builtin_amdgcn_perm(acc, r0, 0x07060302u);
	}
	if (pub_stripe) {
		if (lane == (S_end & 7)) hb = (u32)__builtin_amdgcn_readlane((int)pk2, 63) >> 16;
		const int row = (S_end & ~7) - 128 + lane;
		if (lane <= (S_end & 7) && row >= 0 && row < m) {
			if (out_lds) __hip_atomic_store(&lout[row], (ep << 16) | hb, __ATOMIC_RELAXED, __HIP_MEMORY_SCOPE_WORKGROUP);
			else __hip_atomic_store(&bnd_out[row], (ep << 16) | hb, __ATOMIC_RELAXED, __HIP_MEMORY_SCOPE_AGENT);
		}
	}
	DPT(if (pp == 0 && lane == 0) ctr[sj.ctr + 40] = (u32)(wall_clock64() - T0c); if (pp == PP - 1 && lane == 0) ctr[sj.ctr + 41] = (u32)(wall_clock64() - T0c);)
	const bool one_wg = WPB > 1 && PP <= WPB;
	const int first_p = ((int)bid - sj.first_block) * WPB;
	const int mine = PP - first_p < WPB ? PP - first_p : WPB, n_wg = (PP + WPB - 1) / WPB;
	u32 ticket = 0;
	if (WPB > 1) {
		__builtin_amdgcn_fence(__ATOMIC_RELEASE, "workgroup");
		asm volatile("s_waitcnt vmcnt(0)" ::: "memory");
		if (lane == 0) ticket = __hip_atomic_fetch_add(&s_tick, 1u, __ATOMIC_RELAXED, __HIP_MEMORY_SCOPE_WORKGROUP);
		ticket = (u32)__builtin_amdgcn_readfirstlane((int)ticket);
		if ((int)ticket != mine - 1) return;
		__builtin_amdgcn_fence(__ATOMIC_ACQUIRE, "workgroup");
	}
	if (!one_wg) {
		__builtin_amdgcn_fence(__ATOMIC_RELEASE, "agent");
		asm volatile("s_waitcnt vmcnt(0)" ::: "memory");
		if (lane == 0) ticket = __hip_atomic_fetch_add(&ctr[sj.ctr], 1u, __ATOMIC_RELAXED, __HIP_MEMORY_SCOPE_AGENT);
		ticket = (u32)__builtin_amdgcn_readfirstlane((int)ticket);
		if ((int)ticket != (WPB > 1 ? n_wg : PP) - 1) return;
		if (lane == 0) ctr[sj.ctr] = 0;
		__builtin_amdgcn_fence(__ATOMIC_ACQUIRE, "agent");
	}
	DPT(const unsigned long long T1c = wall_clock64(); int ntile = 0, nrun = 0;)
	uint8_t *rev = revbase + ops_off[sj.job], *op = ops + ops_off[sj.job];
	int i = n - 1, j = m - 1, state = 0, k = 0;
	const int g = lane / DP_LOOK, e = lane - g * DP_LOOK;
	const int dlc = g == 2 ? 0 : -e, drl = g == 0 ? -2 * e : -e;
	constexpr int TB_BLKS = DP_TILE_ROWS / 8, TB_VEC = TB_BLKS * 16 / 64;
	static_assert(TB_VEC == 5, "the prefetched tile is five named registers (an array was kept in scratch: 96 bytes per lane)");
	uint4 pf0 = {0, 0, 0, 0}, pf1 = pf0, pf2 = pf0, pf3 = pf0, pf4 = pf0;
#define PF_EACH(X) X(0, pf0) X(1, pf1) X(2, pf2) X(3, pf3) X(4, pf4)
	int pf_sp = -1, pf_lo = 0, pf_hi = -1;
	const int rl_max = m - 1 + 63;
	const u32 *tile32 = (const u32 *)tile;
	while (i >= 0 && j >= 0) {
		i = __builtin_amdgcn_readfirstlane(i); j = __builtin_amdgcn_readfirstlane(j);
		DPT(ntile++;)
		const int sp = i >> 6, rl_hi = j + (i & 63);
		int rl_lo;
		uint4 *dst = (uint4 *)tile;
		if (sp == pf_sp && rl_hi <= pf_hi && rl_hi - pf_lo >= 64) {
			rl_lo = pf_lo;
			DPT(nrun += 1 << 16;)
#define PF_PUT(Q, R) dst[(Q) * 64 + lane] = R;
			PF_EACH(PF_PUT)
#undef PF_PUT
		} else {
			const int b_hi = rl_hi >> 3, b_lo = b_hi - (TB_BLKS - 1) > 0 ? b_hi - (TB_BLKS - 1) : 0;
			rl_lo = b_lo << 3;
			const uint4 *src = (const uint4 *)(dir + (size_t)sp * pitch + ((size_t)b_lo << 8));
			const int nvec = (b_hi - b_lo + 1) * 16;
#pragma unroll
			for (int q2 = 0; q2 < TB_VEC; q2++) { const int id = q2 * 64 + lane; if (id < nvec) dst[id] = src[id]; }
		}
		pf_sp = -1;
		{
			const int jp = j - ((i & 63) + 1);
			if (sp > 0 && jp >= 0) {
				int hi = jp + 63 + DP_TILE_SLACK; hi = hi < rl_max ? hi : rl_max;
				const int pb_hi = hi >> 3, pb_lo = pb_hi - (TB_BLKS - 1) > 0 ? pb_hi - (TB_BLKS - 1) : 0;
				const uint4 *src = (const uint4 *)(dir + (size_t)(sp - 1) * pitch + ((size_t)pb_lo << 8));
				const int nvec = (pb_hi - pb_lo + 1) * 16;
#define PF_GET(Q, R) { const int id = (Q) * 64 + lane; R = src[id < nvec ? id : 0]; }
				PF_EACH(PF_GET)
#undef PF_GET
				pf_sp = sp - 1; pf_lo = pb_lo << 3; pf_hi = (pb_hi << 3) + 7 < rl_max ? (pb_hi << 3) + 7 : rl_max;
			}
		}
		__builtin_amdgcn_fence(__ATOMIC_RELEASE, "workgroup");
		__builtin_amdgcn_wave_barrier();
		__builtin_amdgcn_fence(__ATOMIC_ACQUIRE, "workgroup");
		for (;;) {
			i = __builtin_amdgcn_readfirstlane(i); j = __builtin_amdgcn_readfirstlane(j);
			state = __builtin_amdgcn_readfirstlane(state); k = __builtin_amdgcn_readfirstlane(k);
			if (i < 0 || j < 0) break;
			const int lc = i - (sp << 6), rl = j + lc;
			if (lc < 0 || rl < rl_lo) break;
			const int lc2 = lc + dlc, rl2 = rl + drl;
			const bool valid = lane < 3 * DP_LOOK && lc2 >= 0 && rl2 >= rl_lo && rl2 - lc2 >= 0;
			u32 tmp = 0xffu;
			if (valid) {
				const u32 nb = (tile32[(((rl2 - rl_lo) >> 3) << 6) + lc2] >> ((((rl2 & 7) >> 2) << 4) + ((3 - (rl2 & 3)) << 2))) & 15u;
				tmp = ((nb & 2u) ? 2u : (nb & 1u)) | ((nb & 0xCu) << 1);
			}
			const u32 cur = (u32)__builtin_amdgcn_readfirstlane((int)tmp);
			const int S = dp_bt_next(state, cur);
			const int isM = S == 0 ? 1 : 0, isD = (S == 1 || S == 3) ? 1 : 0;
			const int gS = isM ? 0 : (isD ? 1 : 2);
			const bool cont = valid && g == gS && (isM ? (tmp & 7) == 0 : (((tmp >> (S + 2)) & 1) != 0 || (int)(tmp & 7) == S));
			const unsigned long long bal = __ballot(cont) >> (gS * DP_LOOK + 1);
			int run = __builtin_ctzll(~bal);
			run = run < DP_LOOK - 1 ? run : DP_LOOK - 1;
			const int L = 1 + run;
			if (lane < L) rev[k + lane] = (uint8_t)(isM ? 'M' : (isD ? 'D' : 'I'));
			k += L; state = S; DPT(nrun++;)
			i -= (isM | isD) ? L : 0; j -= (isM | (1 - isD)) ? L : 0;
		}
	}
	DPT(if (lane == 0) { ctr[sj.ctr + 42] = (u32)(wall_clock64() - T1c); ctr[sj.ctr + 43] = ntile; ctr[sj.ctr + 44] = nrun; ctr[sj.ctr + 45] = (u32)(wall_clock64() - T0c); })
	if (lane == 0) {
		for (; i >= 0; --i) rev[k++] = 'D';
		for (; j >= 0; --j) rev[k++] = 'I';
		ops_len[sj.job] = k;
	}
	k = __builtin_amdgcn_readfirstlane(k);
	__builtin_amdgcn_fence(__ATOMIC_RELEASE, "workgroup");
	asm volatile("s_waitcnt vmcnt(0)" ::: "memory");
	__builtin_amdgcn_fence(__ATOMIC_ACQUIRE, "workgroup");
	for (int q2 = lane; q2 < k; q2 += 64) op[q2] = rev[k - 1 - q2];
}

int launch_stripes(gsa_ctx *c, hipStream_t st, std::vector<LgJob> &large, const uint8_t *pool1, const i64 *off1, const uint8_t *pool2, const i64 *off2,
                   uint8_t *ops, const i64 *ops_off, i32 *ops_len, uint8_t *rev, int err_slot)
{
	if (large.empty()) return GSA_OK;
	i32 *mail = c->d_mail.as<i32>();
	{
		auto by_cells = [](const LgJob &a, const LgJob &b) { const i64 ca = (i64)a.m * a.n, cb = (i64)b.m * b.n; return ca != cb ? ca > cb : a.job < b.job; };
		if (large.size() > 512) std::partial_sort(large.begin(), large.begin() + 256, large.end(), by_cells);
		else std::sort(large.begin(), large.end(), by_cells);
	}
	size_t n_xl = 0, n_top = large.size(), n_hi = large.size();
	{
		auto it0 = std::stable_partition(large.begin(), large.end(), [](const LgJob &g) { return g.m > DP_LDS_M; });
		n_xl = (size_t)(it0 - large.begin());
		if (large.size() >= DP_CLASS_MIN_JOBS) {
			auto it1 = std::stable_partition(it0, large.end(), [](const LgJob &g) { return g.m > DP_CLASS_TOP; });
			auto it = std::stable_partition(it1, large.end(), [](const LgJob &g) { return g.m > DP_CLASS_M; });
			n_top = (size_t)(it1 - large.begin()); n_hi = (size_t)(it - large.begin());
		}
	}
	for (const LgJob &g : large) if ((((g.m + 63) & ~63) + DP_C1_PAD) * 4 > 150 * 1024) return gsa_fail(c, GSA_ERR_LIMIT, "DP reference-side fragment longer than 38000 bases");
	const i64 budget = 12ll << 30;
	size_t first = 0;
	while (first < large.size()) {
		size_t cnt = 0;
		if (c->dp_safe) cnt = 1;
		else { size_t l = first; i64 db = 128; while (l < large.size()) { const i64 cells = (((i64)large[l].n + 63) / 64) * (i64)DP_STRIPE_BYTES(large[l].m); if (l > first && db + cells > budget) break; db += cells + 128; l++; } cnt = l - first; }
		DevBuf &psj = err_slot == M_DPERR3 ? c->p_sj_early : c->p_sj;
		const size_t s0 = std::min(std::max(n_xl, first), first + cnt), stp = std::min(std::max(n_top, first), first + cnt), s1 = std::min(std::max(n_hi, first), first + cnt);
		constexpr int NSEG = 4;
		struct Seg { size_t b, e; int mmax, wpb, mpad, lds_rows; size_t dyn_lds; i32 *b2j; i32 nblocks; } seg[NSEG] = { { first, s0 }, { s0, stp }, { stp, s1 }, { s1, first + cnt } };
		size_t nb_ub = 0;
		for (Seg &sg : seg) {
			sg.mmax = 1;
			for (size_t k = sg.b; k < sg.e; k++) if (large[k].m > sg.mmax) sg.mmax = large[k].m;
			sg.mpad = ((sg.mmax + 63) & ~63) + DP_C1_PAD;
			sg.wpb = sg.mmax <= DP_LDS_M ? 4 : 1;
			sg.lds_rows = (sg.mmax + 15) & ~15;
			sg.dyn_lds = (size_t)sg.mpad * 4 + (sg.wpb > 1 ? (size_t)(sg.wpb - 1) * sg.lds_rows * 4 : 0);
			if (sg.dyn_lds < (size_t)DP_TILE_ROWS * 32) sg.dyn_lds = (size_t)DP_TILE_ROWS * 32;
			for (size_t k = sg.b; k < sg.e; k++) nb_ub += (size_t)((((large[k].n + 63) / 64 + 1) / 2 + sg.wpb - 1) / sg.wpb);
		}
		if (!pin_ensure<char>(c, psj, (cnt + 1) * sizeof(StripeJob) + (nb_ub + 2) * 4)) return GSA_ERR_NOMEM;
		StripeJob *sj = psj.as<StripeJob>();
		i32 *b2j_all = (i32 *)(sj + cnt + 1);
		i64 dbytes = 128, bwords = 0; i32 nctr = NSEG; size_t b2j_used = 0;
		for (Seg &sg : seg) {
			sg.b2j = b2j_all + b2j_used; sg.nblocks = 0;
			for (size_t k = sg.b; k < sg.e; k++) {
				const LgJob &g = large[k];
				const i64 cells = (((i64)g.n + 63) / 64) * (i64)DP_STRIPE_BYTES(g.m);
				StripeJob s; s.job = g.job; s.m = g.m; s.n = g.n; s.P = (g.n + 63) / 64;
				s.diroff = dbytes; dbytes += cells + 128;
				s.bndoff = bwords; bwords += (i64)(s.P - 1) * g.m;
				s.ctr = nctr++; s.first_block = sg.nblocks;
				for (int b = 0; b < ((s.P + 1) / 2 + sg.wpb - 1) / sg.wpb; b++) sg.b2j[sg.nblocks++] = (i32)(k - first);
				sj[k - first] = s;
			}
			b2j_used += (size_t)sg.nblocks;
		}
		const size_t last = first + cnt;
		uint8_t *dir = dev_ensure<uint8_t>(c, c->d_scan2, (size_t)dbytes + 512);
		const size_t bnd_cap0 = c->d_dp_bnd.cap;
		u32 *bnd = dev_ensure<u32>(c, c->d_dp_bnd, (size_t)bwords + 64);
		const size_t ctr_cap0 = c->d_dp_ctr.cap;
		u32 *ctr = dev_ensure<u32>(c, c->d_dp_ctr, (size_t)nctr + 64);
		if (!dir || !bnd || !ctr) return GSA_ERR_NOMEM;
		c->dp_epoch = (c->dp_epoch + 1) & 0xffffu;
		if (c->dp_epoch == 0 || c->d_dp_bnd.cap != bnd_cap0) { GSA_CHECK(c, hipMemsetAsync(bnd, 0, c->d_dp_bnd.cap, st)); if (c->dp_epoch == 0) c->dp_epoch = 1; }
		if (c->d_dp_ctr.cap != ctr_cap0 || c->dp_dirty) { GSA_CHECK(c, hipMemsetAsync(ctr, 0, c->d_dp_ctr.cap, st)); GSA_CHECK(c, hipMemsetAsync(mail + err_slot, 0, 4, st)); c->dp_dirty = false; }
		const bool side = c->opt.dp_side && c->stream_aux[3] && seg[NSEG - 1].nblocks > 0 && (seg[0].nblocks > 0 || seg[1].nblocks > 0 || seg[2].nblocks > 0);
		if (side) { GSA_CHECK(c, hipEventRecord(c->ev[24], st)); GSA_CHECK(c, hipStreamWaitEvent(c->stream_aux[3], c->ev[24], 0)); }
		hipStream_t st_main = st;
		for (int si = 0; si < NSEG; si++) {
			const Seg &sg = seg[si];
			if (sg.nblocks == 0) continue;
			hipStream_t st = (side && si == NSEG - 1) ? c->stream_aux[3] : st_main;
			if (sg.wpb == 4) hipLaunchKernelGGL(k_dp_stripe<4>, dim3((unsigned)sg.nblocks), dim3(256), sg.dyn_lds, st, (const i32 *)sg.b2j, (const StripeJob *)sj, pool1, off1, pool2, off2, dir + 256, bnd, ctr, rev, ops, ops_off, ops_len, c->dp_epoch, (i32)(sg.mpad * 4), (i32)sg.lds_rows, (u32 *)(mail + err_slot), si);
			else hipLaunchKernelGGL(k_dp_stripe<1>, dim3((unsigned)sg.nblocks), dim3(64), sg.dyn_lds, st, (const i32 *)sg.b2j, (const StripeJob *)sj, pool1, off1, pool2, off2, dir + 256, bnd, ctr, rev, ops, ops_off, ops_len, c->dp_epoch, (i32)(sg.mpad * 4), (i32)sg.lds_rows, (u32 *)(mail + err_slot), si);
		}
		if (side) { GSA_CHECK(c, hipEventRecord(c->ev[25], c->stream_aux[3])); GSA_CHECK(c, hipStreamWaitEvent(st, c->ev[25], 0)); }
		GSA_CHECK(c, hipGetLastError());
		DPT(GSA_CHECK(c, hipStreamSynchronize(st)); if (cnt == 1) { u32 hh[6]; hipMemcpy(hh, ctr + sj[0].ctr + 40, 24, hipMemcpyDeviceToHost); fprintf(stderr, "[dp] %d x %d: fwd0 %.1f us  fwdlast %.1f us  traceback %.1f us (tiles %u runs %u)  total %.1f us\n", sj[0].m, sj[0].n, hh[0] * 0.01, hh[1] * 0.01, hh[2] * 0.01, hh[3], hh[4], hh[5] * 0.01); })
		if (last < large.size()) {
			i32 *h = c->h_mail;
			GSA_CHECK(c, hipMemcpyAsync(h, mail, MAIL_N * sizeof(i32), hipMemcpyDeviceToHost, st));
			GSA_CHECK(c, hipStreamSynchronize(st));
			if (h[err_slot]) { c->dp_dirty = c->dp_timeout = true; return gsa_fail(c, GSA_ERR_STATE, "internal: DP stripe hand-off timed out"); }
		}
		first = last;
	}
	return GSA_OK;
}
```

### include/gsa_hip.h

```cpp
#ifndef GSA_HIP_H
#define GSA_HIP_H
#include <stddef.h>
#include <stdint.h>
#ifdef __cplusplus
extern "C" {
#endif

typedef struct gsa_ctx gsa_ctx;

enum {
	GSA_OK = 0,
	GSA_ERR_ARG = -1,
	GSA_ERR_HIP = -2,
	GSA_ERR_NOMEM = -3,
	GSA_ERR_STATE = -4,
	GSA_ERR_LIMIT = -5
};

typedef struct {
	uint64_t primary;
	uint64_t L2[5];
	const uint32_t *bwt;
	uint64_t bwt_words;
	const uint64_t *sa;
// ... 92 lines not shown
int gsa_align_contig_device(gsa_ctx *ctx, const char *d_query, int32_t qlen, gsa_result *out);
int gsa_prefetch_contig(gsa_ctx *ctx, const char *query, int32_t qlen);
int gsa_prefetch_bundle(gsa_ctx *ctx, const char *const *query, const int32_t *qlen, int32_t n);
int gsa_cancel_prefetch(gsa_ctx *ctx);
void *gsa_device_alloc(int device, size_t bytes);
void  gsa_device_free(int device, void *p);
int   gsa_device_upload(int device, void *dst, const void *src, size_t bytes);

typedef int (*gsa_result_fn)(void *user, int32_t contig, const gsa_result *res);
#define GSA_MANY_IN_ORDER 1u
#define GSA_MANY_DEVICE   2u
#define GSA_MANY_NO_SPLIT 4u
#define GSA_MANY_NO_BUNDLE 8u
#define GSA_MANY_NO_PREFETCH 16u
int gsa_align_many(gsa_ctx *const *ctx, int32_t n_ctx, const char *const *query, const int32_t *qlen, int32_t n,
                   uint32_t flags, gsa_result_fn on_result, void *user);

int gsa_align_bundle(gsa_ctx *ctx, const char *const *query, const int32_t *qlen, int32_t n, uint32_t flags, gsa_result *out);

typedef struct { int64_t rpos; int32_t qpos, len, chr, pos, kind, block; } gsa_variant;
typedef struct { int64_t n; const gsa_variant *v; int64_t n_snv, n_ins, n_del; } gsa_variants;
static inline void gsa_variant_alleles(const gsa_variant *v, const char *ref, const char *query,
                                       const char **ref_p, uint32_t *ref_n, const char **alt_p, uint32_t *alt_n)
{
	const char *r = ref + v->rpos, *q = query + v->qpos;
	const uint32_t n = (uint32_t)v->len + 1;
	switch (v->kind) {
	case 1:  *ref_p = r; *ref_n = 1; *alt_p = q; *alt_n = n; break;
	case 2:  *ref_p = r; *ref_n = n; *alt_p = q; *alt_n = 1; break;
	case 3:  *ref_p = q; *ref_n = 1; *alt_p = q; *alt_n = n; break;
	case 4:  *ref_p = r; *ref_n = n; *alt_p = r; *alt_n = 1; break;
	default: *ref_p = r; *ref_n = 1; *alt_p = q; *alt_n = 1; break;
	}
}
int gsa_call_variants(gsa_ctx *ctx, int32_t k, gsa_variants *out);
int gsa_get_variant_timing(gsa_ctx *ctx, double *ms_sum, int64_t *n_calls);
typedef int (*gsa_result_var_fn)(void *user, int32_t contig, const gsa_result *res, const gsa_variants *var);
int gsa_align_many_variants(gsa_ctx *const *ctx, int32_t n_ctx, const char *const *query, const int32_t *qlen, int32_t n,
                            uint32_t flags, gsa_result_var_fn on_result, void *user);

typedef struct { int64_t cig_off; int32_t n_cig; int32_t n_eq, n_x, n_ins, n_del; int32_t _pad; } gsa_block_cigar;
typedef struct { int32_t n_blocks; int64_t n_ops; const gsa_block_cigar *blk; const uint32_t *ops; } gsa_cigars;
#define GSA_CIGAR_INS 1u
#define GSA_CIGAR_DEL 2u
#define GSA_CIGAR_EQ  7u
#define GSA_CIGAR_X   8u
static inline size_t gsa_cigar_string(const uint32_t *ops, int64_t n, char *buf, size_t cap)
{
	static const char letter[16] = { 'M', 'I', 'D', 'N', 'S', 'H', 'P', '=', 'X', '?', '?', '?', '?', '?', '?', '?' };
	size_t at = 0;
	for (int64_t i = 0; i < n; i++) {
		char tmp[12]; int m = 0; uint32_t len = ops[i] >> 4;
		do { tmp[m++] = (char)('0' + len % 10); len /= 10; } while (len);
		while (m) { --m; if (at + 1 < cap) buf[at] = tmp[m]; at++; }
		if (at + 1 < cap) buf[at] = letter[ops[i] & 15u];
		at++;
	}
	if (cap) buf[at < cap ? at : cap - 1] = '\0';
	return at;
}
int gsa_block_cigars(gsa_ctx *ctx, int32_t k, gsa_cigars *out);
int gsa_get_cigar_timing(gsa_ctx *ctx, double *ms_sum, int64_t *n_calls);
typedef struct { int64_t cs_off; int32_t n_cs; int32_t _pad; } gsa_cs_block;
typedef struct { int32_t n_blocks; int64_t n_bytes; const gsa_cs_block *blk; const char *cs; } gsa_cs;
int gsa_block_cs(gsa_ctx *ctx, int32_t k, gsa_cs *out);
int gsa_get_cs_timing(gsa_ctx *ctx, double *ms_sum, int64_t *n_calls);

typedef struct { int32_t idx;
                 int32_t qpos; int32_t block;
                 uint8_t cls, rev; uint16_t n_cover; } gsa_lift_hit;
typedef struct { int64_t n_hits; const gsa_lift_hit *hits; } gsa_lifts;
int gsa_lift_set(gsa_ctx *ctx, const int64_t *pos, int64_t n);
int gsa_lift(gsa_ctx *ctx, int32_t k, gsa_lifts *out);
int gsa_get_lift_timing(gsa_ctx *ctx, double *ms_sum, int64_t *n_calls);

typedef struct { int32_t chr, start, len; uint32_t n_cov, n_eq, n_x, n_del, n_ins; } gsa_track_win;
typedef struct { int64_t n_win; const gsa_track_win *win; } gsa_tracks;
int gsa_track_set(gsa_ctx *ctx, int32_t window);
int gsa_ref_track(gsa_ctx *ctx, int32_t k, gsa_tracks *out);
int gsa_get_track_timing(gsa_ctx *ctx, double *ms_sum, int64_t *n_calls);

typedef struct { int32_t size, dt, dq; } gsa_seg;
typedef struct { int64_t seg_off; int32_t n_seg; int32_t _pad; } gsa_seg_block;
typedef struct { int32_t n_blocks; int64_t n_segs; const gsa_seg_block *blk; const gsa_seg *seg; } gsa_segs;
int gsa_block_segs(gsa_ctx *ctx, int32_t k, gsa_segs *out);
int gsa_get_seg_timing(gsa_ctx *ctx, double *ms_sum, int64_t *n_calls);

#define GSA_PROJ_NO_DUP 1u
typedef struct { int32_t n_blocks; int32_t _pad; int64_t n_cols; } gsa_proj_stat;
int gsa_proj_open(gsa_ctx *ctx, gsa_ctx *share, uint32_t flags);
int gsa_proj_close(gsa_ctx *ctx);
int gsa_proj_clear(gsa_ctx *ctx);
int gsa_project(gsa_ctx *ctx, int32_t k, gsa_proj_stat *out);
int gsa_proj_fetch(gsa_ctx *ctx, int64_t p0, int64_t n, char *text, uint32_t *words);
int gsa_proj_merge(gsa_ctx *ctx, int64_t p0, int64_t n, const uint32_t *words);
int gsa_get_proj_timing(gsa_ctx *ctx, double *ms_sum, int64_t *n_calls);

#define GSA_WANT_VARIANTS 1u
#define GSA_WANT_CIGARS   2u
#define GSA_WANT_CS       4u
#define GSA_WANT_LIFT     16u
#define GSA_WANT_TRACK    32u
#define GSA_WANT_SEGS     64u
#define GSA_WANT_PROJ     128u
typedef struct { const gsa_variants *var; const gsa_cigars *cig; } gsa_extras;
int gsa_extras_cs(const gsa_extras *ex, gsa_cs *out);
int gsa_extras_lift(const gsa_extras *ex, gsa_lifts *out);
int gsa_extras_track(const gsa_extras *ex, gsa_tracks *out);
int gsa_extras_segs(const gsa_extras *ex, gsa_segs *out);
typedef int (*gsa_result_ex_fn)(void *user, int32_t contig, const gsa_result *res, const gsa_extras *ex);
int gsa_align_many_ex(gsa_ctx *const *ctx, int32_t n_ctx, const char *const *query, const int32_t *qlen, int32_t n,
                      uint32_t flags, uint32_t want, gsa_result_ex_fn on_result, void *user);

int gsa_index_sizes(int64_t G, uint64_t *bwt_words, uint64_t *n_sa);
int gsa_build_index(int device, const uint8_t *pac, int64_t G, uint64_t *primary, uint64_t L2[5], uint32_t *bwt, uint64_t *sa);
int gsa_get_index_build_stats(double *ms, int32_t *rounds);

int gsa_seed_chunks(gsa_ctx *ctx, const char *query, int32_t qlen, int32_t chunk_beg, int32_t chunk_end);
int64_t gsa_hit_count(gsa_ctx *ctx);
int gsa_export_hits(gsa_ctx *ctx, uint64_t *keys, uint32_t *vals);
int gsa_import_hits(gsa_ctx *ctx, const uint64_t *keys, const uint32_t *vals, int64_t n);
int gsa_hit_buffers(gsa_ctx *ctx, const uint64_t **keys, const uint32_t **vals);
int gsa_finish_contig(gsa_ctx *ctx, gsa_result *out);

int gsa_set_query(gsa_ctx *ctx, const char *query, int32_t qlen);
int gsa_set_query_device(gsa_ctx *ctx, const char *d_query, int32_t qlen);
int gsa_rewind(gsa_ctx *ctx);
int gsa_run_to(gsa_ctx *ctx, int stage);

int64_t gsa_seed_count(gsa_ctx *ctx);
int  gsa_get_seeds(gsa_ctx *ctx, gsa_seed *out);
int  gsa_group_count(gsa_ctx *ctx);
int  gsa_get_groups(gsa_ctx *ctx, int32_t *beg, int32_t *end);
int  gsa_get_blocks(gsa_ctx *ctx, gsa_result *out);

int gsa_bwt_search_batch(gsa_ctx *ctx, int32_t n, const int32_t *start, const int32_t *stop,
                         int32_t *out_len, int32_t *out_freq, int64_t *out_loc);

int gsa_ksw2_batch(gsa_ctx *ctx, int32_t n_pairs,
                   const char *pool1, const int64_t *off1, const int32_t *len1,
                   const char *pool2, const int64_t *off2, const int32_t *len2,
                   char *ops, const int64_t *ops_off, int32_t *ops_len);

int gsa_gap_similarity_batch(gsa_ctx *ctx, int32_t n, const int32_t *q1, const int32_t *q2,
                             const int64_t *r1, const int64_t *r2, int32_t *similar);

int gsa_get_counters(gsa_ctx *ctx, uint64_t counters[8]);
int gsa_get_timings(gsa_ctx *ctx, float kernel_ms[8]);
int gsa_get_wall_sums(gsa_ctx *ctx, double ms[10], int64_t *n);
int gsa_get_alloc_stats(gsa_ctx *ctx, double *ms, int64_t *n, int64_t *bytes);
int gsa_debug_buffers(gsa_ctx *ctx, int top);
int gsa_set_profiling(gsa_ctx *ctx, int flags);
int gsa_get_seed_stats(gsa_ctx *ctx, uint64_t stats[8]);

#ifdef __cplusplus
}
#endif
#endif
```

Baseline: 36.98 Gbp/s.

## Pair two DP jobs per wave in stripe kernel when it saves wave-steps

Adds a paired-job variant of the DP stripe kernel. One wave computes 64 columns of two different jobs in the two packed 16-bit halves, instead of 128 columns of one job. Jobs in long classes are grouped into units sorted by cell count, and each unit is paired only when that costs fewer lagged wave-steps. Paired and single launches run on separate streams. The boundary hand-off packs two 4-bit halves into one word. It also turns off the high-priority block setting and adds DP stats counters. This adds complexity to the boundary packing and sync, and the per-segment launches double.

```diff
diff --git a/gsalign_amd/capi.py b/gsalign_amd/capi.py
--- a/gsalign_amd/capi.py
+++ b/gsalign_amd/capi.py
@@ -11,7 +11,7 @@
 
 EXPORTS = [
     "gsa_default_params", "gsa_create", "gsa_create_opts", "gsa_reserve_index", "gsa_release_reserved", "gsa_clone", "gsa_clone_to_device", "gsa_host_alloc", "gsa_host_free", "gsa_destroy", "gsa_set_params", "gsa_last_error", "gsa_align_contig", "gsa_align_many", "gsa_align_bundle",
-    "gsa_align_contig_device", "gsa_set_query_device", "gsa_device_alloc", "gsa_device_free", "gsa_device_upload", "gsa_get_seed_stats", "gsa_hit_buffers", "gsa_seed_chunks", "gsa_hit_count", "gsa_export_hits", "gsa_import_hits", "gsa_finish_contig",
+    "gsa_align_contig_device", "gsa_set_query_device", "gsa_device_alloc", "gsa_device_free", "gsa_device_upload", "gsa_get_seed_stats", "gsa_get_dp_stats", "gsa_hit_buffers", "gsa_seed_chunks", "gsa_hit_count", "gsa_export_hits", "gsa_import_hits", "gsa_finish_contig",
     "gsa_set_query", "gsa_rewind", "gsa_run_to", "gsa_seed_count", "gsa_get_seeds", "gsa_group_count", "gsa_get_groups", "gsa_get_blocks",
     "gsa_bwt_search_batch", "gsa_ksw2_batch", "gsa_gap_similarity_batch", "gsa_get_counters", "gsa_get_timings", "gsa_set_profiling", "gsa_bind_host_thread",
     "gsa_prefetch_contig", "gsa_prefetch_bundle", "gsa_cancel_prefetch", "gsa_get_wall_sums", "gsa_get_alloc_stats", "gsa_debug_buffers", "gsa_set_option", "gsa_host_register", "gsa_host_unregister",
@@ -425,7 +425,7 @@
 
 class Aligner:
 
-    ENV_OPTIONS = ("split_min", "bundle_contig", "bundle_cap", "seed_budget", "dp_lane", "seed_mode", "pd_bitmap", "walk_chain_min", "pd_two_level_min", "pres_from_kmer", "pd_bytes", "sweep_shape", "dp_side", "dp_safe", "dp_fake_timeout")
+    ENV_OPTIONS = ("split_min", "bundle_contig", "bundle_cap", "seed_budget", "dp_lane", "seed_mode", "pd_bitmap", "walk_chain_min", "pd_two_level_min", "pres_from_kmer", "pd_bytes", "sweep_shape", "dp_side", "dp_pair", "dp_safe", "dp_fake_timeout")
 
     def _options_from_env(self):
         for name in self.ENV_OPTIONS:
@@ -555,6 +555,11 @@
         self._ck(self.lib.gsa_get_seed_stats(self.ctx, _p(st, C.c_uint64)))
         return st
 
+    def dp_stats(self) -> np.ndarray:
+        st = np.zeros(4, np.uint64)
+        self._ck(self.lib.gsa_get_dp_stats(self.ctx, _p(st, C.c_uint64)))
+        return st
+
     def _params(self, slen=15, ind=25, clr=200, alen=200, idy=70, sen=0, one=0) -> Params:
         return Params(slen, ind, clr, alen, idy, sen, one)
 
diff --git a/gsalign_amd/csrc/gsa_api.hip b/gsalign_amd/csrc/gsa_api.hip
--- a/gsalign_amd/csrc/gsa_api.hip
+++ b/gsalign_amd/csrc/gsa_api.hip
@@ -436,5 +436,6 @@
 }
 int gsa_get_counters(gsa_ctx *c, uint64_t counters[8]) { if (!c) return GSA_ERR_ARG; memcpy(counters, c->counters, sizeof(c->counters)); return GSA_OK; }
 int gsa_get_timings(gsa_ctx *c, float ms[8]) { if (!c) return GSA_ERR_ARG; memcpy(ms, c->kernel_ms, sizeof(c->kernel_ms)); if (c->prof_seed && !c->profiling) ms[6] = (float)c->acc_seed_ms; return GSA_OK; }
+int gsa_get_dp_stats(gsa_ctx *c, uint64_t st[4]) { if (!c) return GSA_ERR_ARG; memcpy(st, c->dp_stats, sizeof(c->dp_stats)); return GSA_OK; }
 int gsa_get_seed_stats(gsa_ctx *c, uint64_t st[8]) { if (!c) return GSA_ERR_ARG; memcpy(st, c->dbg, sizeof(c->dbg)); return GSA_OK; }
 }
diff --git a/gsalign_amd/csrc/gsa_create.hip b/gsalign_amd/csrc/gsa_create.hip
--- a/gsalign_amd/csrc/gsa_create.hip
+++ b/gsalign_amd/csrc/gsa_create.hip
@@ -460,6 +460,7 @@
 	else if (k == "seed_lhop") { if (value != 0 && (!in(16, 1 << 16) || (value & (value - 1)))) return gsa_fail(c, GSA_ERR_ARG, "seed_lhop: 0 or a power of two >= 16"); c->opt.seed_lhop = (int)value; }
 	else if (k == "pd_bitmap") c->opt.pd_bitmap = value != 0;
 	else if (k == "dp_side") c->opt.dp_side = value != 0;
+	else if (k == "dp_pair") { if (!in(0, 3)) return gsa_fail(c, GSA_ERR_ARG, "dp_pair: 0 never, 1 where it costs fewer wave-steps in a long class, 2 always, 3 where it costs fewer wave-steps"); c->opt.dp_pair = (int)value; }
 	else if (k == "pd_two_level_min") { if (!in(0, BIG)) return gsa_fail(c, GSA_ERR_ARG, "pd_two_level_min: >= 0 blocks"); c->opt.pd_two_level_min = value; }
 	else if (k == "pd_bytes") { if (!in(0, 2)) return gsa_fail(c, GSA_ERR_ARG, "pd_bytes: 0 never, 1 by the hit count, 2 always"); c->opt.pd_bytes = (int)value; }
 	else if (k == "pres_from_kmer") c->opt.pres_from_kmer = value != 0;
diff --git a/gsalign_amd/csrc/gsa_ctx.h b/gsalign_amd/csrc/gsa_ctx.h
--- a/gsalign_amd/csrc/gsa_ctx.h
+++ b/gsalign_amd/csrc/gsa_ctx.h
@@ -62,6 +62,7 @@
 	int pd_bitmap = 1;
 	int sweep_shape = -1;
 	int dp_side = 0;
+	int dp_pair = 1;
 	int64_t walk_chain_min = 100000;
 	int64_t pd_two_level_min = 2000000;
 	int pd_bytes = 1;
@@ -99,6 +100,7 @@
 	double wall_ms[10] = {0, 0, 0, 0, 0, 0, 0, 0, 0, 0}; int64_t wall_n = 0;
 	double acc_seed_ms = 0.0;
 	u64 counters[8] = {};
+	u64 dp_stats[4] = {};
 
 	DevBuf d_bwt, d_bwt_ref, d_occ_base, d_sa, d_ref, d_chr_end, d_chr_of_end;
 	std::vector<i64> h_chr_end, h_chr_fwd; std::vector<i32> h_chr_of_end, h_chr_len;
diff --git a/gsalign_amd/csrc/k_dp_stripe.hip b/gsalign_amd/csrc/k_dp_stripe.hip
--- a/gsalign_amd/csrc/k_dp_stripe.hip
+++ b/gsalign_amd/csrc/k_dp_stripe.hip
@@ -20,8 +20,9 @@
 #define DP_CLASS_M 768
 #define DP_CLASS_TOP 1536
 #define DP_CLASS_MIN_JOBS 4096
+#define DP_PAIR_MIN_JOBS 4096
 #ifndef DP_PRIO_BLOCKS
-#define DP_PRIO_BLOCKS 96
+#define DP_PRIO_BLOCKS 0
 #endif
 #define DP_LDS_M 3968
 
@@ -37,7 +38,10 @@
 __device__ __forceinline__ u32 pk_shl(u32 a, u32 sh) { return U1(V2(a) << V2(sh)); }
 #define DP_OPAQUE(X) asm volatile("" : "+v"(X))
 
-template <int WPB>
+__device__ __forceinline__ u32 dp_pack4(u32 h) { return (h & 0xfu) | ((h >> 4) & 0xf0u) | ((h >> 8) & 0xf00u) | ((h >> 12) & 0xf000u); }
+__device__ __forceinline__ u32 dp_unpack4(u32 g) { return (g & 0xfu) | ((g & 0xf0u) << 4) | ((g & 0xf00u) << 8) | ((g & 0xf000u) << 12); }
+
+template <int WPB, int SBS>
 __global__ void __launch_bounds__(64 * WPB) k_dp_stripe(const i32 *__restrict__ blk2job, const StripeJob *__restrict__ sjobs, const uint8_t *__restrict__ pool1, const i64 *__restrict__ off1,
                                                    const uint8_t *__restrict__ pool2, const i64 *__restrict__ off2, uint8_t *dirbase, u32 *bndbase, u32 *ctr,
                                                    uint8_t *revbase, uint8_t *ops, const i64 *__restrict__ ops_off, i32 *ops_len, u32 ep, i32 lds_c1, i32 lds_rows, u32 *err, i32 tick_slot)
@@ -53,21 +57,27 @@
 	}
 	__syncthreads();
 	const u32 bid = s_bid;
-	if (bid < DP_PRIO_BLOCKS) __builtin_amdgcn_s_setprio(3);
+	if (DP_PRIO_BLOCKS > 0 && bid < (u32)DP_PRIO_BLOCKS) __builtin_amdgcn_s_setprio(3);
 	const StripeJob sj = sjobs[blk2job[bid]];
+	const StripeJob sy = SBS ? sjobs[blk2job[bid] + 1] : sj;
 	const int lane = threadIdx.x & 63, wave = threadIdx.x >> 6;
-	const int m = sj.m, n = sj.n, P = sj.P, PP = (P + 1) >> 1;
+	const int m = sj.m, n = sj.n, P = sj.P, PP = SBS ? (P > sy.P ? P : sy.P) : (P + 1) >> 1;
+	const int mB = SBS ? sy.m : m, nB = SBS ? sy.n : n;
+	const int mv = SBS ? (m > mB ? m : mB) : m;
 	const int pp = ((int)bid - sj.first_block) * WPB + wave;
 	const uint8_t *s1 = pool1 + off1[sj.job], *s2 = pool2 + off2[sj.job];
+	const uint8_t *s1B = SBS ? pool1 + off1[sy.job] : s1, *s2B = SBS ? pool2 + off2[sy.job] : s2;
 	const size_t pitch = (size_t)DP_STRIPE_BYTES(m);
 	const int nblk = (m + 63 + 7) >> 3;
+	const int nblkB = SBS ? (mB + 63 + 7) >> 3 : nblk;
 	uint8_t *dir = dirbase + sj.diroff;
-	u32 *bnd_in = bndbase + sj.bndoff + (size_t)(pp - 1) * m, *bnd_out = bndbase + sj.bndoff + (size_t)pp * m;
+	u32 *bnd_in = bndbase + sj.bndoff + (size_t)(pp - 1) * mv, *bnd_out = bndbase + sj.bndoff + (size_t)pp * mv;
+	constexpr int LEAD = SBS ? 64 : 128;
 	{
-		int fe = (m + DP_C1_PAD + 63) & ~63; fe = fe < (lds_c1 >> 2) ? fe : (lds_c1 >> 2);
+		int fe = (mv + DP_C1_PAD + 63) & ~63; fe = fe < (lds_c1 >> 2) ? fe : (lds_c1 >> 2);
 		for (int t = threadIdx.x; t < fe; t += 64 * WPB) {
-			const int j = t - 128, jb = j - 64;
-			const u32 ca = (j >= 0 && j < m) ? (u32)gsa_nt4(s1[j]) : 4u, cb = (jb >= 0 && jb < m) ? (u32)gsa_nt4(s1[jb]) : 4u;
+			const int j = t - LEAD, jb = j - (SBS ? 0 : 64);
+			const u32 ca = (j >= 0 && j < m) ? (u32)gsa_nt4(s1[j]) : 4u, cb = (jb >= 0 && jb < (SBS ? mB : m)) ? (u32)gsa_nt4((SBS ? s1B : s1)[jb]) : 4u;
 			C2[t] = (ca < 4 ? ca : 0x0cu) | 0x0c000c00u | ((cb < 4 ? 4u + cb : 0x0cu) << 16);
 		}
 	}
@@ -75,34 +85,40 @@
 	if (WPB > 1) for (int t = threadIdx.x; t < (WPB - 1) * lds_rows; t += 64 * WPB) lds_bnd[t] = 0;
 	u32 *lin = lds_bnd + (size_t)(wave > 0 ? wave - 1 : 0) * lds_rows, *lout = lds_bnd + (size_t)(wave < WPB - 1 ? wave : 0) * lds_rows;
 	const bool out_lds = WPB > 1 && wave < WPB - 1;
-	const int tA = pp * 128 + lane, tB = tA + 64;
-	const bool hasB = 2 * pp + 1 < P;
-	const int WpB = !hasB ? 0 : (n - pp * 128 - 64 < 64 ? n - pp * 128 - 64 : 64);
-	const int WpA = n - pp * 128 < 64 ? n - pp * 128 : 64;
-	const int cqA = tA < n ? gsa_nt4(s2[tA]) : 4, cqB = tB < n ? gsa_nt4(s2[tB]) : 4;
+	const int tA = SBS ? pp * 64 + lane : pp * 128 + lane, tB = SBS ? tA : tA + 64;
+	const bool hasA = SBS ? pp < P : true, hasB = SBS ? pp < sy.P : 2 * pp + 1 < P;
+	const int restA = SBS ? n - pp * 64 : n - pp * 128, restB = SBS ? nB - pp * 64 : n - pp * 128 - 64;
+	const int WpB = !hasB ? 0 : (restB < 64 ? restB : 64);
+	const int WpA = restA < 64 ? restA : 64;
+	const int cqA = tA < n ? gsa_nt4(s2[tA]) : 4, cqB = tB < nB ? gsa_nt4(s2B[tB]) : 4;
 	u32 tblA = 0, tblB = 0;
 #pragma unroll
 	for (int cc = 0; cc < 4; cc++) {
 		tblA |= (u32)(cqA == 4 ? 0 : (cqA == cc ? 7 ^ 6 : 5 ^ 6)) << (8 * cc);
 		tblB |= (u32)(cqB == 4 ? 0 : (cqB == cc ? 7 ^ 6 : 5 ^ 6)) << (8 * cc);
 	}
-	const u32 uinit2 = (tA ? 2u : 0u) | (2u << 16);
+	const u32 uinit2 = SBS ? (tA ? 0x00020002u : 0u) : (tA ? 2u : 0u) | (2u << 16);
 	u32 u2 = uinit2, y2 = 0;
 	u32 bin = 0, gnext = 0;
 	__syncthreads();
 	if (pp >= PP) return;
-	const int S_end = hasB ? 64 + m + WpB - 1 : m + WpA - 1;
+	const int S_endA = hasA ? m + WpA - 1 : 0, S_endB = hasB ? mB + WpB - 1 : 0;
+	const int S_end = SBS ? (S_endA > S_endB ? S_endA : S_endB) : (hasB ? 64 + m + WpB - 1 : m + WpA - 1);
+	const int mw = SBS ? ((hasA ? m : 0) > (hasB ? mB : 0) ? (hasA ? m : 0) : (hasB ? mB : 0)) : m;
+	const int mpub = SBS ? ((pp + 1 < P ? m : 0) > (pp + 1 < sy.P ? mB : 0) ? (pp + 1 < P ? m : 0) : (pp + 1 < sy.P ? mB : 0)) : m;
+	const int nblk_lo = SBS ? ((hasA ? nblk : 0x7fffffff) < (hasB ? nblkB : 0x7fffffff) ? (hasA ? nblk : 0x7fffffff) : (hasB ? nblkB : 0x7fffffff)) : nblk;
 	DPT(const unsigned long long T0c = wall_clock64();)
-	u32 *dirA = (u32 *)(dir + (size_t)(2 * pp) * pitch), *dirB = (u32 *)(dir + (size_t)(2 * pp + 1) * pitch);
+	u32 *dirA = (u32 *)(dir + (size_t)(SBS ? pp : 2 * pp) * pitch);
+	u32 *dirB = SBS ? (u32 *)(dirbase + sy.diroff + (size_t)pp * DP_STRIPE_BYTES(mB)) : (u32 *)(dir + (size_t)(2 * pp + 1) * pitch);
 	if (pp > 0) {
-		const int row = (lane & (DP_G - 1)) < m ? (lane & (DP_G - 1)) : m - 1;
+		const int row = (lane & (DP_G - 1)) < mw ? (lane & (DP_G - 1)) : mw - 1;
 		gnext = (WPB > 1 && wave > 0) ? __hip_atomic_load(&lin[row], __ATOMIC_RELAXED, __HIP_MEMORY_SCOPE_WORKGROUP) : __hip_atomic_load(&bnd_in[row], __ATOMIC_RELAXED, __HIP_MEMORY_SCOPE_AGENT);
 	}
 	asm volatile("" :: "v"(gnext));
 	const bool pub_stripe = pp < PP - 1;
 	u32 pk2 = 0;
 	u32 hb = 0;
-	const u32 selx = lane ? 0x0c060c04u : 0x0c040c00u, selv = lane ? 0x0c070c05u : 0x0c050c01u;
+	const u32 selx = lane ? 0x0c060c04u : (SBS ? 0x0c020c00u : 0x0c040c00u), selv = lane ? 0x0c070c05u : (SBS ? 0x0c030c01u : 0x0c050c01u);
 	u32 acc = 0, r0 = 0;
 	u32 c1 = 0x00010001u, c2 = 0x00020002u, c4 = 0x00040004u, c7 = 0x00070007u, c16 = 0x00100010u;
 	DP_OPAQUE(c1); DP_OPAQUE(c2); DP_OPAQUE(c4); DP_OPAQUE(c7); DP_OPAQUE(c16);
@@ -113,11 +129,11 @@
 	{                                                                                                           \
 		const int s_ = s0 + (K2);                                                                               \
 		if (((K2) & (DP_G - 1)) == 0) {                                                                         \
-			if ((MODE) == 0) bin = (s_ == 0 && lane == 0) ? 0u : 0x200u;     \
-			else if (s_ < m) {                                                                                  \
+			if ((MODE) == 0) bin = (s_ == 0 && lane == 0) ? 0u : (SBS ? 0x02000200u : 0x200u);     \
+			else if (s_ < mw) {                                                                                 \
 				 \
 				const int row = s_ + (lane & (DP_G - 1));                                                       \
-				const bool need = lane < DP_G && row < m;                                                       \
+				const bool need = lane < DP_G && row < mw;                                                      \
 				u32 g = gnext;                                                                                  \
 				if (!__all(!need || (g >> 16) == ep)) {       \
 					u32 spins = 0; const unsigned long long t_wait0 = wall_clock64();                          \
@@ -127,9 +143,9 @@
 						if (need) g = DP_LOADG(MODE, row);                                                      \
 					} while (!__all(!need || (g >> 16) == ep));                                                  \
 				}                                                                                               \
-				bin = g & 0xffffu;                                                                              \
+				bin = SBS ? dp_unpack4(g) : g & 0xffffu;                                                                      \
 				 \
-				const int rown = row + DP_G < m ? row + DP_G : m - 1;                                           \
+				const int rown = row + DP_G < mw ? row + DP_G : mw - 1;                                         \
 				gnext = DP_LOADG(MODE, rown);                                                                   \
 			}                                                                                                   \
 		}                                                                                                       \
@@ -137,7 +153,7 @@
 		                          \
 		const u32 bin0 = (u32)__builtin_amdgcn_readlane((int)bin, (K2) & (DP_G - 1));                           \
 		const u32 rot = (u32)__builtin_amdgcn_mov_dpp((int)pk2, 0x13C, 0xf, 0xf, true);                         \
-		WL(hb, (u32)__builtin_amdgcn_readlane((int)pk2, 63) >> 16, (K2) & 7)       \
+		WL(hb, (u32)__builtin_amdgcn_readlane((int)pk2, 63) >> (SBS ? 0 : 16), (K2) & 7)       \
 		const u32 x1 = __builtin_amdgcn_perm(rot, bin0, selx), v1 = __builtin_amdgcn_perm(rot, bin0, selv);     \
 		const u32 z0 = __builtin_amdgcn_perm(tblB, tblA, (WSEL)) ^ 0x00060006u;                                 \
 		const u32 a = pk_add(x1, v1), b = pk_add(y2, u2);                                                       \
@@ -152,31 +168,31 @@
 		u2 = un; y2 = yb;                                                                                       \
 		pk2 = __builtin_amdgcn_perm(vn, xa, 0x06020400u);       \
 		if (GUARD) {                                                                                            \
-			const u32 keep = (lane <= s_ ? 0xffffu : 0u) | (lane <= s_ - 64 ? 0xffff0000u : 0u);               \
+			const u32 keep = (lane <= s_ ? 0xffffu : 0u) | (lane <= s_ - (SBS ? 0 : 64) ? 0xffff0000u : 0u); \
 			u2 = (u2 & keep) | (uinit2 & ~keep); y2 &= keep;                                                    \
 		}                                                                                                       \
 		if (((K2) & 7) == 3) r0 = acc;                                                                  \
 		if (((K2) & 7) == 7) {                                                                                  \
 			const int blk = s_ >> 3;                                                                            \
-			if (!(GUARD) || blk < nblk) dirA[((size_t)blk << 6) + lane] = __builtin_amdgcn_perm(acc, r0, 0x05040100u); \
-			if (hasB && (!(GUARD) || (blk >= 8 && blk - 8 < nblk))) dirB[((size_t)(blk - 8) << 6) + lane] = __builtin_amdgcn_perm(acc, r0, 0x07060302u); \
+			if (hasA && (!(GUARD) || blk < nblk)) dirA[((size_t)blk << 6) + lane] = __builtin_amdgcn_perm(acc, r0, 0x05040100u); \
+			if (hasB && (!(GUARD) || (blk >= LEAD / 8 - 8 && blk - (LEAD / 8 - 8) < nblkB))) dirB[((size_t)(blk - (LEAD / 8 - 8)) << 6) + lane] = __builtin_amdgcn_perm(acc, r0, 0x07060302u); \
 		}                                                                                                       \
-		if (((K2) & 7) == 7 && pub_stripe && s_ >= 135) {                                                       \
-			   \
-			const int row = s_ - 135 + lane;                                                                    \
-			if (lane < 8 && row < m) {                                                                          \
-				if (out_lds) __hip_atomic_store(&lout[row], (ep << 16) | hb, __ATOMIC_RELAXED, __HIP_MEMORY_SCOPE_WORKGROUP); \
-				else __hip_atomic_store(&bnd_out[row], (ep << 16) | hb, __ATOMIC_RELAXED, __HIP_MEMORY_SCOPE_AGENT); \
+		if (((K2) & 7) == 7 && pub_stripe && s_ >= LEAD + 7) {                                                  \
+			 \
+			const int row = s_ - (LEAD + 7) + lane;                                                             \
+			if (lane < 8 && row < mpub) {                                                                       \
+				if (out_lds) __hip_atomic_store(&lout[row], (ep << 16) | (SBS ? dp_pack4(hb) : hb), __ATOMIC_RELAXED, __HIP_MEMORY_SCOPE_WORKGROUP); \
+				else __hip_atomic_store(&bnd_out[row], (ep << 16) | (SBS ? dp_pack4(hb) : hb), __ATOMIC_RELAXED, __HIP_MEMORY_SCOPE_AGENT); \
 			}                                                                                                   \
 		}                                                                                                       \
 	}
 #define DP_LOOP(MODE)                                                                                           \
 	for (int s0 = 0; s0 < S_end; s0 += 16) {                                                                    \
-		const u32 *crow = C2 + 128 + s0 - lane;                                  \
+		const u32 *crow = C2 + LEAD + s0 - lane;                                 \
 		if (s0 + 16 <= S_end) {                                                                                 \
 			u32 w[16];                                                                                          \
 			_Pragma("unroll") for (int k2 = 0; k2 < 16; k2++) w[k2] = crow[k2];                                   \
-			if (s0 >= 128 && s0 + 16 <= 8 * nblk) {                                                             \
+			if (s0 >= LEAD && s0 + 16 <= 8 * nblk_lo) {                                                         \
 				 \
 				DP_STEP(0, MODE, w[0], 0, DP_WL_LIT) DP_STEP(1, MODE, w[1], 0, DP_WL_LIT) DP_STEP(2, MODE, w[2], 0, DP_WL_LIT) DP_STEP(3, MODE, w[3], 0, DP_WL_LIT) DP_STEP(4, MODE, w[4], 0, DP_WL_LIT) DP_STEP(5, MODE, w[5], 0, DP_WL_LIT) DP_STEP(6, MODE, w[6], 0, DP_WL_LIT) DP_STEP(7, MODE, w[7], 0, DP_WL_LIT) \
 				DP_STEP(8, MODE, w[8], 0, DP_WL_LIT) DP_STEP(9, MODE, w[9], 0, DP_WL_LIT) DP_STEP(10, MODE, w[10], 0, DP_WL_LIT) DP_STEP(11, MODE, w[11], 0, DP_WL_LIT) DP_STEP(12, MODE, w[12], 0, DP_WL_LIT) DP_STEP(13, MODE, w[13], 0, DP_WL_LIT) DP_STEP(14, MODE, w[14], 0, DP_WL_LIT) DP_STEP(15, MODE, w[15], 0, DP_WL_LIT) \
@@ -196,15 +212,15 @@
 		if (S_end & 3) acc = pk_shl(acc, (u32)(4 * (4 - (S_end & 3))) * 0x00010001u);
 		if ((S_end & 7) < 4) r0 = acc;
 		const int blk = S_end >> 3;
-		if (blk < nblk) dirA[((size_t)blk << 6) + lane] = __builtin_amdgcn_perm(acc, r0, 0x05040100u);
-		if (hasB && blk >= 8 && blk - 8 < nblk) dirB[((size_t)(blk - 8) << 6) + lane] = __builtin_amdgcn_perm(acc, r0, 0x07060302u);
+		if (hasA && blk < nblk) dirA[((size_t)blk << 6) + lane] = __builtin_amdgcn_perm(acc, r0, 0x05040100u);
+		if (hasB && blk >= LEAD / 8 - 8 && blk - (LEAD / 8 - 8) < nblkB) dirB[((size_t)(blk - (LEAD / 8 - 8)) << 6) + lane] = __builtin_amdgcn_perm(acc, r0, 0x07060302u);
 	}
 	if (pub_stripe) {
-		if (lane == (S_end & 7)) hb = (u32)__builtin_amdgcn_readlane((int)pk2, 63) >> 16;
-		const int row = (S_end & ~7) - 128 + lane;
-		if (lane <= (S_end & 7) && row >= 0 && row < m) {
-			if (out_lds) __hip_atomic_store(&lout[row], (ep << 16) | hb, __ATOMIC_RELAXED, __HIP_MEMORY_SCOPE_WORKGROUP);
-			else __hip_atomic_store(&bnd_out[row], (ep << 16) | hb, __ATOMIC_RELAXED, __HIP_MEMORY_SCOPE_AGENT);
+		if (lane == (S_end & 7)) hb = (u32)__builtin_amdgcn_readlane((int)pk2, 63) >> (SBS ? 0 : 16);
+		const int row = (S_end & ~7) - LEAD + lane;
+		if (lane <= (S_end & 7) && row >= 0 && row < mpub) {
+			if (out_lds) __hip_atomic_store(&lout[row], (ep << 16) | (SBS ? dp_pack4(hb) : hb), __ATOMIC_RELAXED, __HIP_MEMORY_SCOPE_WORKGROUP);
+			else __hip_atomic_store(&bnd_out[row], (ep << 16) | (SBS ? dp_pack4(hb) : hb), __ATOMIC_RELAXED, __HIP_MEMORY_SCOPE_AGENT);
 		}
 	}
 	DPT(if (pp == 0 && lane == 0) ctr[sj.ctr + 40] = (u32)(wall_clock64() - T0c); if (pp == PP - 1 && lane == 0) ctr[sj.ctr + 41] = (u32)(wall_clock64() - T0c);)
@@ -230,92 +246,132 @@
 		__builtin_amdgcn_fence(__ATOMIC_ACQUIRE, "agent");
 	}
 	DPT(const unsigned long long T1c = wall_clock64(); int ntile = 0, nrun = 0;)
-	uint8_t *rev = revbase + ops_off[sj.job], *op = ops + ops_off[sj.job];
-	int i = n - 1, j = m - 1, state = 0, k = 0;
-	const int g = lane / DP_LOOK, e = lane - g * DP_LOOK;
-	const int dlc = g == 2 ? 0 : -e, drl = g == 0 ? -2 * e : -e;
-	constexpr int TB_BLKS = DP_TILE_ROWS / 8, TB_VEC = TB_BLKS * 16 / 64;
-	static_assert(TB_VEC == 5, "the prefetched tile is five named registers (an array was kept in scratch: 96 bytes per lane)");
-	uint4 pf0 = {0, 0, 0, 0}, pf1 = pf0, pf2 = pf0, pf3 = pf0, pf4 = pf0;
+	int h = 0;
+walk_back:
+	{
+		const int wm = h ? mB : m, wn = h ? nB : n;
+		const i32 wjob = h ? sy.job : sj.job;
+		const uint8_t *wdir = h ? dirbase + sy.diroff : dir;
+		const size_t wpitch = (size_t)DP_STRIPE_BYTES(wm);
+		uint8_t *rev = revbase + ops_off[wjob], *op = ops + ops_off[wjob];
+		int i = wn - 1, j = wm - 1, state = 0, k = 0;
+		const int g = lane / DP_LOOK, e = lane - g * DP_LOOK;
+		const int dlc = g == 2 ? 0 : -e, drl = g == 0 ? -2 * e : -e;
+		constexpr int TB_BLKS = DP_TILE_ROWS / 8, TB_VEC = TB_BLKS * 16 / 64;
+		static_assert(TB_VEC == 5, "the prefetched tile is five named registers (an array was kept in scratch: 96 bytes per lane)");
+		uint4 pf0 = {0, 0, 0, 0}, pf1 = pf0, pf2 = pf0, pf3 = pf0, pf4 = pf0;
 #define PF_EACH(X) X(0, pf0) X(1, pf1) X(2, pf2) X(3, pf3) X(4, pf4)
-	int pf_sp = -1, pf_lo = 0, pf_hi = -1;
-	const int rl_max = m - 1 + 63;
-	const u32 *tile32 = (const u32 *)tile;
-	while (i >= 0 && j >= 0) {
-		i = __builtin_amdgcn_readfirstlane(i); j = __builtin_amdgcn_readfirstlane(j);
-		DPT(ntile++;)
-		const int sp = i >> 6, rl_hi = j + (i & 63);
-		int rl_lo;
-		uint4 *dst = (uint4 *)tile;
-		if (sp == pf_sp && rl_hi <= pf_hi && rl_hi - pf_lo >= 64) {
-			rl_lo = pf_lo;
-			DPT(nrun += 1 << 16;)
+		int pf_sp = -1, pf_lo = 0, pf_hi = -1;
+		const int rl_max = wm - 1 + 63;
+		const u32 *tile32 = (const u32 *)tile;
+		while (i >= 0 && j >= 0) {
+			i = __builtin_amdgcn_readfirstlane(i); j = __builtin_amdgcn_readfirstlane(j);
+			DPT(ntile++;)
+			const int sp = i >> 6, rl_hi = j + (i & 63);
+			int rl_lo;
+			uint4 *dst = (uint4 *)tile;
+			if (sp == pf_sp && rl_hi <= pf_hi && rl_hi - pf_lo >= 64) {
+				rl_lo = pf_lo;
+				DPT(nrun += 1 << 16;)
 #define PF_PUT(Q, R) dst[(Q) * 64 + lane] = R;
-			PF_EACH(PF_PUT)
+				PF_EACH(PF_PUT)
 #undef PF_PUT
-		} else {
-			const int b_hi = rl_hi >> 3, b_lo = b_hi - (TB_BLKS - 1) > 0 ? b_hi - (TB_BLKS - 1) : 0;
-			rl_lo = b_lo << 3;
-			const uint4 *src = (const uint4 *)(dir + (size_t)sp * pitch + ((size_t)b_lo << 8));
-			const int nvec = (b_hi - b_lo + 1) * 16;
+			} else {
+				const int b_hi = rl_hi >> 3, b_lo = b_hi - (TB_BLKS - 1) > 0 ? b_hi - (TB_BLKS - 1) : 0;
+				rl_lo = b_lo << 3;
+				const uint4 *src = (const uint4 *)(wdir + (size_t)sp * wpitch + ((size_t)b_lo << 8));
+				const int nvec = (b_hi - b_lo + 1) * 16;
 #pragma unroll
-			for (int q2 = 0; q2 < TB_VEC; q2++) { const int id = q2 * 64 + lane; if (id < nvec) dst[id] = src[id]; }
-		}
-		pf_sp = -1;
-		{
-			const int jp = j - ((i & 63) + 1);
-			if (sp > 0 && jp >= 0) {
-				int hi = jp + 63 + DP_TILE_SLACK; hi = hi < rl_max ? hi : rl_max;
-				const int pb_hi = hi >> 3, pb_lo = pb_hi - (TB_BLKS - 1) > 0 ? pb_hi - (TB_BLKS - 1) : 0;
-				const uint4 *src = (const uint4 *)(dir + (size_t)(sp - 1) * pitch + ((size_t)pb_lo << 8));
-				const int nvec = (pb_hi - pb_lo + 1) * 16;
+				for (int q2 = 0; q2 < TB_VEC; q2++) { const int id = q2 * 64 + lane; if (id < nvec) dst[id] = src[id]; }
+			}
+			pf_sp = -1;
+			{
+				const int jp = j - ((i & 63) + 1);
+				if (sp > 0 && jp >= 0) {
+					int hi = jp + 63 + DP_TILE_SLACK; hi = hi < rl_max ? hi : rl_max;
+					const int pb_hi = hi >> 3, pb_lo = pb_hi - (TB_BLKS - 1) > 0 ? pb_hi - (TB_BLKS - 1) : 0;
+					const uint4 *src = (const uint4 *)(wdir + (size_t)(sp - 1) * wpitch + ((size_t)pb_lo << 8));
+					const int nvec = (pb_hi - pb_lo + 1) * 16;
 #define PF_GET(Q, R) { const int id = (Q) * 64 + lane; R = src[id < nvec ? id : 0]; }
-				PF_EACH(PF_GET)
+					PF_EACH(PF_GET)
 #undef PF_GET
-				pf_sp = sp - 1; pf_lo = pb_lo << 3; pf_hi = (pb_hi << 3) + 7 < rl_max ? (pb_hi << 3) + 7 : rl_max;
+					pf_sp = sp - 1; pf_lo = pb_lo << 3; pf_hi = (pb_hi << 3) + 7 < rl_max ? (pb_hi << 3) + 7 : rl_max;
+				}
 			}
-		}
+			__builtin_amdgcn_fence(__ATOMIC_RELEASE, "workgroup");
+			__builtin_amdgcn_wave_barrier();
+			__builtin_amdgcn_fence(__ATOMIC_ACQUIRE, "workgroup");
+			for (;;) {
+				i = __builtin_amdgcn_readfirstlane(i); j = __builtin_amdgcn_readfirstlane(j);
+				state = __builtin_amdgcn_readfirstlane(state); k = __builtin_amdgcn_readfirstlane(k);
+				if (i < 0 || j < 0) break;
+				const int lc = i - (sp << 6), rl = j + lc;
+				if (lc < 0 || rl < rl_lo) break;
+				const int lc2 = lc + dlc, rl2 = rl + drl;
+				const bool valid = lane < 3 * DP_LOOK && lc2 >= 0 && rl2 >= rl_lo && rl2 - lc2 >= 0;
+				u32 tmp = 0xffu;
+				if (valid) {
+					const u32 nb = (tile32[(((rl2 - rl_lo) >> 3) << 6) + lc2] >> ((((rl2 & 7) >> 2) << 4) + ((3 - (rl2 & 3)) << 2))) & 15u;
+					tmp = ((nb & 2u) ? 2u : (nb & 1u)) | ((nb & 0xCu) << 1);
+				}
+				const u32 cur = (u32)__builtin_amdgcn_readfirstlane((int)tmp);
+				const int S = dp_bt_next(state, cur);
+				const int isM = S == 0 ? 1 : 0, isD = (S == 1 || S == 3) ? 1 : 0;
+				const int gS = isM ? 0 : (isD ? 1 : 2);
+				const bool cont = valid && g == gS && (isM ? (tmp & 7) == 0 : (((tmp >> (S + 2)) & 1) != 0 || (int)(tmp & 7) == S));
+				const unsigned long long bal = __ballot(cont) >> (gS * DP_LOOK + 1);
+				int run = __builtin_ctzll(~bal);
+				run = run < DP_LOOK - 1 ? run : DP_LOOK - 1;
+				const int L = 1 + run;
+				if (lane < L) rev[k + lane] = (uint8_t)(isM ? 'M' : (isD ? 'D' : 'I'));
+				k += L; state = S; DPT(nrun++;)
+				i -= (isM | isD) ? L : 0; j -= (isM | (1 - isD)) ? L : 0;
+			}
+		}
+		DPT(if (lane == 0) { ctr[sj.ctr + 42] = (u32)(wall_clock64() - T1c); ctr[sj.ctr + 43] = ntile; ctr[sj.ctr + 44] = nrun; ctr[sj.ctr + 45] = (u32)(wall_clock64() - T0c); })
+		if (lane == 0) {
+			for (; i >= 0; --i) rev[k++] = 'D';
+			for (; j >= 0; --j) rev[k++] = 'I';
+			ops_len[wjob] = k;
+		}
+		k = __builtin_amdgcn_readfirstlane(k);
 		__builtin_amdgcn_fence(__ATOMIC_RELEASE, "workgroup");
-		__builtin_amdgcn_wave_barrier();
+		asm volatile("s_waitcnt vmcnt(0)" ::: "memory");
 		__builtin_amdgcn_fence(__ATOMIC_ACQUIRE, "workgroup");
-		for (;;) {
-			i = __builtin_amdgcn_readfirstlane(i); j = __builtin_amdgcn_readfirstlane(j);
-			state = __builtin_amdgcn_readfirstlane(state); k = __builtin_amdgcn_readfirstlane(k);
-			if (i < 0 || j < 0) break;
-			const int lc = i - (sp << 6), rl = j + lc;
-			if (lc < 0 || rl < rl_lo) break;
-			const int lc2 = lc + dlc, rl2 = rl + drl;
-			const bool valid = lane < 3 * DP_LOOK && lc2 >= 0 && rl2 >= rl_lo && rl2 - lc2 >= 0;
-			u32 tmp = 0xffu;
-			if (valid) {
-				const u32 nb = (tile32[(((rl2 - rl_lo) >> 3) << 6) + lc2] >> ((((rl2 & 7) >> 2) << 4) + ((3 - (rl2 & 3)) << 2))) & 15u;
-				tmp = ((nb & 2u) ? 2u : (nb & 1u)) | ((nb & 0xCu) << 1);
-			}
-			const u32 cur = (u32)__builtin_amdgcn_readfirstlane((int)tmp);
-			const int S = dp_bt_next(state, cur);
-			const int isM = S == 0 ? 1 : 0, isD = (S == 1 || S == 3) ? 1 : 0;
-			const int gS = isM ? 0 : (isD ? 1 : 2);
-			const bool cont = valid && g == gS && (isM ? (tmp & 7) == 0 : (((tmp >> (S + 2)) & 1) != 0 || (int)(tmp & 7) == S));
-			const unsigned long long bal = __ballot(cont) >> (gS * DP_LOOK + 1);
-			int run = __builtin_ctzll(~bal);
-			run = run < DP_LOOK - 1 ? run : DP_LOOK - 1;
-			const int L = 1 + run;
-			if (lane < L) rev[k + lane] = (uint8_t)(isM ? 'M' : (isD ? 'D' : 'I'));
-			k += L; state = S; DPT(nrun++;)
-			i -= (isM | isD) ? L : 0; j -= (isM | (1 - isD)) ? L : 0;
-		}
-	}
-	DPT(if (lane == 0) { ctr[sj.ctr + 42] = (u32)(wall_clock64() - T1c); ctr[sj.ctr + 43] = ntile; ctr[sj.ctr + 44] = nrun; ctr[sj.ctr + 45] = (u32)(wall_clock64() - T0c); })
-	if (lane == 0) {
-		for (; i >= 0; --i) rev[k++] = 'D';
-		for (; j >= 0; --j) rev[k++] = 'I';
-		ops_len[sj.job] = k;
-	}
-	k = __builtin_amdgcn_readfirstlane(k);
-	__builtin_amdgcn_fence(__ATOMIC_RELEASE, "workgroup");
-	asm volatile("s_waitcnt vmcnt(0)" ::: "memory");
-	__builtin_amdgcn_fence(__ATOMIC_ACQUIRE, "workgroup");
-	for (int q2 = lane; q2 < k; q2 += 64) op[q2] = rev[k - 1 - q2];
+		for (int q2 = lane; q2 < k; q2 += 64) op[q2] = rev[k - 1 - q2];
+	}
+	if (SBS && h == 0) { h = 1; goto walk_back; }
+}
+
+static i64 dp_steps_lagged(int m, int n)
+{
+	const int P = (n + 63) / 64; i64 s = 0;
+	for (int pp = 0; 2 * pp < P; pp++) s += 2 * pp + 1 < P ? 64 + m + std::min(n - pp * 128 - 64, 64) - 1 : m + std::min(n - pp * 128, 64) - 1;
+	return s;
+}
+static i64 dp_steps_pair(int mx, int nx, int my, int ny)
+{
+	const int PX = (nx + 63) / 64, PY = (ny + 63) / 64; i64 s = 0;
+	for (int p = 0; p < std::max(PX, PY); p++) s += std::max(p < PX ? mx + std::min(nx - p * 64, 64) - 1 : 0, p < PY ? my + std::min(ny - p * 64, 64) - 1 : 0);
+	return s;
+}
+struct DpUnit { i64 cells; size_t x; long long y; };
+static void dp_make_units(std::vector<LgJob> &large, size_t b, size_t e, int mode, std::vector<DpUnit> &units)
+{
+	units.clear();
+	auto cells = [&](size_t k) { return (i64)large[k].m * large[k].n; };
+	if (mode == 0 || e - b < 2) { for (size_t k = b; k < e; k++) units.push_back({ cells(k), k, -1 }); return; }
+	std::sort(large.begin() + b, large.begin() + e, [](const LgJob &p, const LgJob &q) {
+		const int Pp = (p.n + 63) / 64, Pq = (q.n + 63) / 64;
+		return Pp != Pq ? Pp > Pq : (p.m != q.m ? p.m > q.m : p.job < q.job); });
+	for (size_t k = b; k < e; ) {
+		const bool pair = k + 1 < e && (mode == 2 || dp_steps_pair(large[k].m, large[k].n, large[k + 1].m, large[k + 1].n) < dp_steps_lagged(large[k].m, large[k].n) + dp_steps_lagged(large[k + 1].m, large[k + 1].n));
+		if (pair) { units.push_back({ cells(k) + cells(k + 1), k, (long long)(k + 1) }); k += 2; }
+		else { units.push_back({ cells(k), k, -1 }); k++; }
+	}
+	auto by_cells = [&](const DpUnit &p, const DpUnit &q) { return p.cells != q.cells ? p.cells > q.cells : large[p.x].job < large[q.x].job; };
+	if (units.size() > 512) std::partial_sort(units.begin(), units.begin() + 256, units.end(), by_cells);
+	else std::sort(units.begin(), units.end(), by_cells);
 }
 
 int launch_stripes(gsa_ctx *c, hipStream_t st, std::vector<LgJob> &large, const uint8_t *pool1, const i64 *off1, const uint8_t *pool2, const i64 *off2,
@@ -348,7 +404,7 @@
 		DevBuf &psj = err_slot == M_DPERR3 ? c->p_sj_early : c->p_sj;
 		const size_t s0 = std::min(std::max(n_xl, first), first + cnt), stp = std::min(std::max(n_top, first), first + cnt), s1 = std::min(std::max(n_hi, first), first + cnt);
 		constexpr int NSEG = 4;
-		struct Seg { size_t b, e; int mmax, wpb, mpad, lds_rows; size_t dyn_lds; i32 *b2j; i32 nblocks; } seg[NSEG] = { { first, s0 }, { s0, stp }, { stp, s1 }, { s1, first + cnt } };
+		struct Seg { size_t b, e; int mmax, wpb, mpad, lds_rows; size_t dyn_lds; i32 *b2j[2]; i32 nblocks[2]; std::vector<DpUnit> units; } seg[NSEG] = { { first, s0 }, { s0, stp }, { stp, s1 }, { s1, first + cnt } };
 		size_t nb_ub = 0;
 		for (Seg &sg : seg) {
 			sg.mmax = 1;
@@ -358,25 +414,38 @@
 			sg.lds_rows = (sg.mmax + 15) & ~15;
 			sg.dyn_lds = (size_t)sg.mpad * 4 + (sg.wpb > 1 ? (size_t)(sg.wpb - 1) * sg.lds_rows * 4 : 0);
 			if (sg.dyn_lds < (size_t)DP_TILE_ROWS * 32) sg.dyn_lds = (size_t)DP_TILE_ROWS * 32;
-			for (size_t k = sg.b; k < sg.e; k++) nb_ub += (size_t)((((large[k].n + 63) / 64 + 1) / 2 + sg.wpb - 1) / sg.wpb);
+			for (size_t k = sg.b; k < sg.e; k++) nb_ub += (size_t)(((large[k].n + 63) / 64 + sg.wpb - 1) / sg.wpb);
+			int mode = sg.wpb == 4 ? c->opt.dp_pair : 0;
+			if (mode == 1 && sg.e - sg.b < DP_PAIR_MIN_JOBS) mode = 0;
+			dp_make_units(large, sg.b, sg.e, mode == 3 ? 1 : mode, sg.units);
+			for (const DpUnit &u : sg.units) { c->dp_stats[0] += u.y >= 0 ? 2 : 1; c->dp_stats[1] += u.y >= 0 ? 2 : 0; }
 		}
 		if (!pin_ensure<char>(c, psj, (cnt + 1) * sizeof(StripeJob) + (nb_ub + 2) * 4)) return GSA_ERR_NOMEM;
 		StripeJob *sj = psj.as<StripeJob>();
 		i32 *b2j_all = (i32 *)(sj + cnt + 1);
-		i64 dbytes = 128, bwords = 0; i32 nctr = NSEG; size_t b2j_used = 0;
+		i64 dbytes = 128, bwords = 0; i32 nctr = 2 * NSEG; size_t b2j_used = 0, nsj = 0;
 		for (Seg &sg : seg) {
-			sg.b2j = b2j_all + b2j_used; sg.nblocks = 0;
-			for (size_t k = sg.b; k < sg.e; k++) {
-				const LgJob &g = large[k];
-				const i64 cells = (((i64)g.n + 63) / 64) * (i64)DP_STRIPE_BYTES(g.m);
-				StripeJob s; s.job = g.job; s.m = g.m; s.n = g.n; s.P = (g.n + 63) / 64;
-				s.diroff = dbytes; dbytes += cells + 128;
-				s.bndoff = bwords; bwords += (i64)(s.P - 1) * g.m;
-				s.ctr = nctr++; s.first_block = sg.nblocks;
-				for (int b = 0; b < ((s.P + 1) / 2 + sg.wpb - 1) / sg.wpb; b++) sg.b2j[sg.nblocks++] = (i32)(k - first);
-				sj[k - first] = s;
+			for (int form = 0; form < 2; form++) {
+				sg.b2j[form] = b2j_all + b2j_used; sg.nblocks[form] = 0;
+				for (const DpUnit &u : sg.units) {
+					if ((u.y >= 0) != (form == 1)) continue;
+					const int nj = form ? 2 : 1;
+					StripeJob s[2];
+					for (int q = 0; q < nj; q++) {
+						const LgJob &g = large[q ? (size_t)u.y : u.x];
+						const i64 cells = (((i64)g.n + 63) / 64) * (i64)DP_STRIPE_BYTES(g.m);
+						s[q].job = g.job; s[q].m = g.m; s[q].n = g.n; s[q].P = (g.n + 63) / 64;
+						s[q].diroff = dbytes; dbytes += cells + 128;
+						s[q].bndoff = 0; s[q].ctr = 0; s[q].first_block = sg.nblocks[form];
+					}
+					const int waves = form ? std::max(s[0].P, s[1].P) : (s[0].P + 1) / 2, rows = form ? std::max(s[0].m, s[1].m) : s[0].m;
+					s[0].bndoff = bwords; bwords += (i64)((form ? waves : s[0].P) - 1) * rows;
+					s[0].ctr = nctr++;
+					for (int b = 0; b < (waves + sg.wpb - 1) / sg.wpb; b++) sg.b2j[form][sg.nblocks[form]++] = (i32)nsj;
+					for (int q = 0; q < nj; q++) sj[nsj++] = s[q];
+				}
+				b2j_used += (size_t)sg.nblocks[form];
 			}
-			b2j_used += (size_t)sg.nblocks;
 		}
 		const size_t last = first + cnt;
 		uint8_t *dir = dev_ensure<uint8_t>(c, c->d_scan2, (size_t)dbytes + 512);
@@ -388,17 +457,24 @@
 		c->dp_epoch = (c->dp_epoch + 1) & 0xffffu;
 		if (c->dp_epoch == 0 || c->d_dp_bnd.cap != bnd_cap0) { GSA_CHECK(c, hipMemsetAsync(bnd, 0, c->d_dp_bnd.cap, st)); if (c->dp_epoch == 0) c->dp_epoch = 1; }
 		if (c->d_dp_ctr.cap != ctr_cap0 || c->dp_dirty) { GSA_CHECK(c, hipMemsetAsync(ctr, 0, c->d_dp_ctr.cap, st)); GSA_CHECK(c, hipMemsetAsync(mail + err_slot, 0, 4, st)); c->dp_dirty = false; }
-		const bool side = c->opt.dp_side && c->stream_aux[3] && seg[NSEG - 1].nblocks > 0 && (seg[0].nblocks > 0 || seg[1].nblocks > 0 || seg[2].nblocks > 0);
-		if (side) { GSA_CHECK(c, hipEventRecord(c->ev[24], st)); GSA_CHECK(c, hipStreamWaitEvent(c->stream_aux[3], c->ev[24], 0)); }
+		auto blocks_of = [&](int si) { return seg[si].nblocks[0] + seg[si].nblocks[1]; };
+		const bool side = c->opt.dp_side && c->stream_aux[3] && blocks_of(NSEG - 1) > 0 && (blocks_of(0) > 0 || blocks_of(1) > 0 || blocks_of(2) > 0);
+		bool beside = false;
+		for (const Seg &sg : seg) if (sg.nblocks[0] > 0 && sg.nblocks[1] > 0 && c->stream_aux[3]) beside = true;
+		if (side || beside) { GSA_CHECK(c, hipEventRecord(c->ev[24], st)); GSA_CHECK(c, hipStreamWaitEvent(c->stream_aux[3], c->ev[24], 0)); }
 		hipStream_t st_main = st;
 		for (int si = 0; si < NSEG; si++) {
 			const Seg &sg = seg[si];
-			if (sg.nblocks == 0) continue;
-			hipStream_t st = (side && si == NSEG - 1) ? c->stream_aux[3] : st_main;
-			if (sg.wpb == 4) hipLaunchKernelGGL(k_dp_stripe<4>, dim3((unsigned)sg.nblocks), dim3(256), sg.dyn_lds, st, (const i32 *)sg.b2j, (const StripeJob *)sj, pool1, off1, pool2, off2, dir + 256, bnd, ctr, rev, ops, ops_off, ops_len, c->dp_epoch, (i32)(sg.mpad * 4), (i32)sg.lds_rows, (u32 *)(mail + err_slot), si);
-			else hipLaunchKernelGGL(k_dp_stripe<1>, dim3((unsigned)sg.nblocks), dim3(64), sg.dyn_lds, st, (const i32 *)sg.b2j, (const StripeJob *)sj, pool1, off1, pool2, off2, dir + 256, bnd, ctr, rev, ops, ops_off, ops_len, c->dp_epoch, (i32)(sg.mpad * 4), (i32)sg.lds_rows, (u32 *)(mail + err_slot), si);
-		}
-		if (side) { GSA_CHECK(c, hipEventRecord(c->ev[25], c->stream_aux[3])); GSA_CHECK(c, hipStreamWaitEvent(st, c->ev[25], 0)); }
+			hipStream_t st_seg = (side && si == NSEG - 1) ? c->stream_aux[3] : st_main;
+			hipStream_t st = (beside && sg.nblocks[1] > 0) ? c->stream_aux[3] : st_seg;
+			c->dp_stats[2] += sg.nblocks[0] > 0; c->dp_stats[3] += sg.nblocks[1] > 0;
+			if (sg.nblocks[0] > 0) {
+				if (sg.wpb == 4) hipLaunchKernelGGL((k_dp_stripe<4, 0>), dim3((unsigned)sg.nblocks[0]), dim3(256), sg.dyn_lds, st, (const i32 *)sg.b2j[0], (const StripeJob *)sj, pool1, off1, pool2, off2, dir + 256, bnd, ctr, rev, ops, ops_off, ops_len, c->dp_epoch, (i32)(sg.mpad * 4), (i32)sg.lds_rows, (u32 *)(mail + err_slot), 2 * si);
+				else hipLaunchKernelGGL((k_dp_stripe<1, 0>), dim3((unsigned)sg.nblocks[0]), dim3(64), sg.dyn_lds, st, (const i32 *)sg.b2j[0], (const StripeJob *)sj, pool1, off1, pool2, off2, dir + 256, bnd, ctr, rev, ops, ops_off, ops_len, c->dp_epoch, (i32)(sg.mpad * 4), (i32)sg.lds_rows, (u32 *)(mail + err_slot), 2 * si);
+			}
+			if (sg.nblocks[1] > 0) hipLaunchKernelGGL((k_dp_stripe<4, 1>), dim3((unsigned)sg.nblocks[1]), dim3(256), sg.dyn_lds, st_seg, (const i32 *)sg.b2j[1], (const StripeJob *)sj, pool1, off1, pool2, off2, dir + 256, bnd, ctr, rev, ops, ops_off, ops_len, c->dp_epoch, (i32)(sg.mpad * 4), (i32)sg.lds_rows, (u32 *)(mail + err_slot), 2 * si + 1);
+		}
+		if (side || beside) { GSA_CHECK(c, hipEventRecord(c->ev[25], c->stream_aux[3])); GSA_CHECK(c, hipStreamWaitEvent(st, c->ev[25], 0)); }
 		GSA_CHECK(c, hipGetLastError());
 		DPT(GSA_CHECK(c, hipStreamSynchronize(st)); if (cnt == 1) { u32 hh[6]; hipMemcpy(hh, ctr + sj[0].ctr + 40, 24, hipMemcpyDeviceToHost); fprintf(stderr, "[dp] %d x %d: fwd0 %.1f us  fwdlast %.1f us  traceback %.1f us (tiles %u runs %u)  total %.1f us\n", sj[0].m, sj[0].n, hh[0] * 0.01, hh[1] * 0.01, hh[2] * 0.01, hh[3], hh[4], hh[5] * 0.01); })
 		if (last < large.size()) {
diff --git a/include/gsa_hip.h b/include/gsa_hip.h
--- a/include/gsa_hip.h
+++ b/include/gsa_hip.h
@@ -268,6 +268,7 @@
 int gsa_debug_buffers(gsa_ctx *ctx, int top);
 int gsa_set_profiling(gsa_ctx *ctx, int flags);
 int gsa_get_seed_stats(gsa_ctx *ctx, uint64_t stats[8]);
+int gsa_get_dp_stats(gsa_ctx *ctx, uint64_t stats[4]);
 
 #ifdef __cplusplus
 }
```

New measurement: 38.71 Gbp/s (median of 6 runs). 1.05x the previous value.
